# cmower/optas

Hardware: AMD Instinct MI355X
Metric: MPC solves/sec (KUKA 7-DoF, T=50) (higher is better)
Workload: dtype f64; 1 GPU; figure_eight_plan T=50 KUKA LWR end_effector_ball (BASELINE configs[1]) x 262144 perturbed instances per GPU (qc0 + U(-0.1,0.1)^7, seed=qc), solved to reduced-gradient tol 1e-08, max_iter 300; batch_per_gpu=262144, global_batch=262144, T=50, parallelism=dp1 (instances sharded, one RCCL broadcast of constants), rccl_world=1, hessian=hybrid, streams_per_gpu=2

## Files before the change

include/optas_hip.h:

```cpp
#ifndef OPTAS_HIP_H
#define OPTAS_HIP_H

#include <stddef.h>

#ifdef __cplusplus
extern "C" {
#endif

#define OH_ABI_VERSION 8

#define OH_MAX_CHAIN 16
#define OH_MAX_T 256

enum {
  OH_OK = 0,
  OH_ERR_INVALID = 1,
  OH_ERR_HIP = 2,
  OH_ERR_STATE = 3
};

enum {
  OH_STATUS_CONVERGED = 0,
  OH_STATUS_MAX_ITER = 1,
  OH_STATUS_NUMERICAL = 2,
// ... 164 lines not shown
typedef struct oh_handle oh_handle;

int oh_create(const oh_problem_desc* desc, oh_handle** out);

int oh_create_pointmass(const oh_pointmass_desc* desc, oh_handle** out);

int oh_create_qp(const oh_qp_desc* desc, oh_handle** out);

int oh_qp_set_tape(oh_handle* h, const oh_tape_desc* tape);

int oh_create_tape(const oh_tape_desc* desc, oh_handle** out);

int oh_tape_probe(oh_handle* h, int B, const double* x, const double* p, int n_regs, const int* regs, double* val, const double* seeds, double* adj,
                  double* grad);

int oh_tape_phi(oh_handle* h, int B, const double* x, const double* p, const double* lam, const double* mu, double rho, double* merit, double* f, double* rows,
                double* grad, double* cmax, double* meas);

int oh_tape_set_metric(oh_handle* h, const double* H0);

int oh_tape_compile(const oh_tape_desc* desc, size_t* code_bytes, char* source, size_t source_cap, size_t* source_len);

int oh_create_torque(const oh_torque_desc* desc, oh_handle** out);

int oh_create_ik(const oh_ik_desc* desc, oh_handle** out);

int oh_set_constants(oh_handle* h, const oh_chain* chain);
int oh_set_constants_device(oh_handle* h, const void* d_chain, size_t nbytes);

#define OH_COMM_ID_BYTES 128
int oh_comm_unique_id(char* id );
int oh_comm_init(int rank, int world, const char* id );
int oh_comm_broadcast_constants(oh_handle* h, int root);
int oh_comm_barrier(void);
int oh_comm_allreduce_max(double* value);
int oh_comm_allreduce_sum(double* value);
int oh_comm_allgather(const void* d_send, void* d_recv, size_t bytes);
int oh_comm_destroy(void);
int oh_comm_info(int* rank, int* world);
int oh_get_constants(oh_handle* h, oh_chain* out);

int oh_set_guards(oh_handle* h, const oh_guards* guards);

int oh_solve(oh_handle* h, int B, const double* x0, const double* p, double* x, double* f, double* kkt,
             int* iters, int* status);

int oh_get_flag(oh_handle* h, const char* name, int* value);

int oh_set_option(oh_handle* h, const char* name, double value);
int oh_get_option(oh_handle* h, const char* name, double* value);

int oh_max_batch(oh_handle* h, int* out);

int oh_solve_device(oh_handle* h, int B, const void* d_x0, const void* d_p, void* d_x, void* d_f, void* d_kkt,
                    void* d_iters, void* d_status);

int oh_pm_rollout(oh_handle* h, int B, int n_ticks, int advance, double ramp, const double* state0, const double* obs_table, double* states,
                  double* f, int* iters, int* status);

int oh_tq_rollout(oh_handle* h, int B, int n_ticks, int advance, double mu_warm, const double* state0, const double* goal_table, double* states,
                  double* tau0, double* f, int* iters, int* status);

int oh_get_multipliers(oh_handle* h, int B, double* lam_h);

int oh_fk_jac(oh_handle* h, int N, const double* q, double* pose, double* J);
int oh_fk_jac_device(oh_handle* h, int N, const void* d_q, void* d_pose, void* d_J);

int oh_set_dynamics(oh_handle* h, const oh_dynamics* dyn);
int oh_rnea(oh_handle* h, int N, const double* q, const double* qd, const double* qdd, double* tau);
int oh_rnea_device(oh_handle* h, int N, const void* d_q, const void* d_qd, const void* d_qdd, void* d_tau);
int oh_rnea_jac(oh_handle* h, int N, const double* q, const double* qd, const double* qdd, double* J);
int oh_rnea_hess(oh_handle* h, int N, const double* q, const double* qd, const double* qdd, const double* c, double* H);

int oh_fk_jac_soa_device(oh_handle* h, int N, const void* d_q, void* d_pose, void* d_J);

typedef struct oh_link_out {
  double *pos, *rot, *quat, *rpy, *axis, *Jg, *Ja;
} oh_link_out;
int oh_set_link_frames(oh_handle* h, const oh_chain* link, const oh_chain* base);
int oh_link_kin(oh_handle* h, int N, const double* q, const double* axis3, const oh_link_out* out);
int oh_link_kin_device(oh_handle* h, int N, const void* d_q, const double* axis3, const oh_link_out* d_out_soa);

int oh_set_profiling(oh_handle* h, int enable);
int oh_get_timing(oh_handle* h, double* out11);

enum { OH_SPECIALIZE_NEVER = 0, OH_SPECIALIZE_ALWAYS = 1, OH_SPECIALIZE_AUTO = 2 };
int oh_specialize(oh_handle* h);
int oh_specialize_compile(const oh_chain* chain, double* info2);
int oh_specialize_info(oh_handle* h, double* info4);
int oh_kernel_info_handle(oh_handle* h, const char* kernel, int* out5);

int oh_device_count(int* n);
int oh_set_device(int index);
int oh_device_malloc(void** ptr, size_t nbytes);
int oh_device_free(void* ptr);
int oh_memcpy_h2d(void* dst, const void* src, size_t nbytes);
int oh_memcpy_d2h(void* dst, const void* src, size_t nbytes);
int oh_device_synchronize(void);
int oh_event_timer_start(oh_handle* h);
int oh_event_timer_stop(oh_handle* h, double* ms);

int oh_kernel_info(const char* kernel, int* out5);

const char* oh_last_error(void);
const char* oh_version(void);
int oh_abi_version(void);
void oh_destroy(oh_handle* h);

#ifdef __cplusplus
}
#endif
#endif
```

optas_amd/backend.py:

```python
from __future__ import annotations

import ctypes as C
import os
from dataclasses import dataclass
from typing import Optional

import numpy as np

from . import _lib


@dataclass
class BatchResult:
    x: np.ndarray
    f: np.ndarray
    kkt: np.ndarray
    iters: np.ndarray
    status: np.ndarray


class _OptionsMixin:

    def set_option(self, name: str, value: float):
        _lib.set_option(self._h, name, value)
        return self

    def set_options(self, options=None, **kw):
        for k, v in {**(options or {}), **kw}.items():
            self.set_option(k, v)
        return self

    def get_option(self, name: str) -> float:
        return _lib.get_option(self._h, name)


class _SolveMixin(_OptionsMixin):

    def solve(self, x0: np.ndarray, p: np.ndarray) -> "BatchResult":
        lib = _lib.load()
        x0 = _lib.as_f64(x0)
        p = _lib.as_f64(p)
        if x0.ndim == 1:
            x0 = x0.reshape(1, -1)
        if p.ndim == 1:
            p = p.reshape(1, -1)
        B = x0.shape[0]
        assert x0.shape == (B, self.nx), f"x0 must be (B, {self.nx})"
        assert p.shape == (B, self.np_), f"p must be (B, {self.np_})"
        chunk = getattr(self, "max_batch", None)
        if chunk and B > chunk:
            parts = [self.solve(x0[i : i + chunk], p[i : i + chunk]) for i in range(0, B, chunk)]
            return BatchResult(*(np.concatenate([getattr(r, k) for r in parts]) for k in ("x", "f", "kkt", "iters", "status")))
        x = np.empty((B, self.nx))
        f = np.empty(B)
        kkt = np.empty((B, 3))
        iters = np.empty(B, dtype=np.int32)
        status = np.empty(B, dtype=np.int32)
        _lib.check(
            lib.oh_solve(self._h, B, _lib._ptr(x0), _lib._ptr(p), _lib._ptr(x), _lib._ptr(f), _lib._ptr(kkt), _lib._ptr(iters), _lib._ptr(status)),
            "oh_solve",
        )
        return BatchResult(x, f, kkt, iters, status)

    def solve_device(self, B: int, d_x0, d_p, d_x, d_f, d_kkt, d_iters, d_status) -> None:
        g = lambda b: None if b is None else b.ptr
        _lib.check(
            _lib.load().oh_solve_device(self._h, int(B), g(d_x0), g(d_p), g(d_x), g(d_f), g(d_kkt), g(d_iters), g(d_status)),
            "oh_solve_device",
        )

    def solve_ms(self) -> float:
        out = (C.c_double * 11)()
        _lib.check(_lib.load().oh_get_timing(self._h, out), "oh_get_timing")
        return out[4]

    def set_profiling(self, on: bool) -> None:
        _lib.check(_lib.load().oh_set_profiling(self._h, 1 if on else 0), "oh_set_profiling")

    def close(self) -> None:
        if getattr(self, "_h", None):
            _lib.load().oh_destroy(self._h)
            self._h = None

    def __del__(self):
        try:
            self.close()
        except Exception:
            pass


class PointMassBackend(_SolveMixin):

    def __init__(self, T=20, dt=0.05, w_acc=0.0025 / 20, ylim=1.5, vlim=1.0, safe=0.3, max_iter=100, tol=1e-8, track_final_only=False, w_vel=0.0,
                 fix_final_velocity=False):
        lib = _lib.load()
        self.T = int(T)
        self.nx, self.np_ = 4 * self.T, 4 + 4 * self.T
        desc = _lib.oh_pointmass_desc(T=self.T, dt=float(dt), w_acc=float(w_acc), ylim=float(ylim), vlim=float(vlim), safe=float(safe),
                                      max_iter=int(max_iter), tol=float(tol), track_final_only=1 if track_final_only else 0, w_vel=float(w_vel),
                                      fix_final_velocity=1 if fix_final_velocity else 0)
        self._h = C.c_void_p()
        _lib.check(lib.oh_create_pointmass(C.byref(desc), C.byref(self._h)), "oh_create_pointmass")

    def rollout(self, state0: np.ndarray, obs_table: np.ndarray, n_ticks: int, advance: int = 2, ramp: float = 0.032):
        state0 = _lib.as_f64(state0).reshape(-1, 4)
        B = state0.shape[0]
        need = n_ticks * advance + self.T
        obs_table = _lib.as_f64(obs_table).reshape(-1, 2)
        assert obs_table.shape[0] >= need, f"obs_table needs {need} rows"
        obs_table = np.ascontiguousarray(obs_table[:need])
        states = np.empty((n_ticks + 1, B, 4))
        f = np.empty((n_ticks, B))
        iters = np.empty((n_ticks, B), dtype=np.int32)
        status = np.empty((n_ticks, B), dtype=np.int32)
        _lib.check(
            _lib.load().oh_pm_rollout(self._h, B, int(n_ticks), int(advance), float(ramp), _lib._ptr(state0), _lib._ptr(obs_table), _lib._ptr(states),
                                      _lib._ptr(f), _lib._ptr(iters), _lib._ptr(status)),
            "oh_pm_rollout",
        )
        return states, f, iters, status


class TapeBackend(_SolveMixin):

    def __init__(self, tape, max_iter=2000, tol=1e-6, tol_feas=1e-9, rho0=10.0, jit=True, wave=True, options=None, keep_regs=None, metric=False):
        self.nx, self.np_ = int(tape.nx), max(1, int(tape.np_))
        self.kept_regs = None if keep_regs is None else np.asarray(keep_regs, dtype=np.int32)
        self._np_real = int(tape.np_)
        self._h = None
        self._h0 = None
        if isinstance(metric, np.ndarray):
            self._h0 = np.ascontiguousarray(metric, dtype=np.float64).reshape(self.nx, self.nx)
        elif metric and int(tape.nx) > 48 and int((options or {}).get("tape_lbfgs", -1)) != 0:
            from .tape import quadratic_cost_metric

            self._h0 = quadratic_cost_metric(tape)
        want_wave = bool(wave) and int(tape.nx) > 48 and float((options or {}).get("tape_wave", 1)) != 0.0
        if want_wave:
            from .tape import Tape, rebalance_sums

            if keep_regs is None:
                bal, kept = rebalance_sums(tape), None
            else:
                nk = len(self.kept_regs)
                tmp = rebalance_sums(Tape(tape.op, tape.a, tape.b, tape.c, tape.out_cost, np.concatenate([tape.out_rows, self.kept_regs]).astype(np.int32),
                                          tape.n_ineq, tape.n_eq + nk, tape.nx, tape.np_))
                bal = Tape(tmp.op, tmp.a, tmp.b, tmp.c, tmp.out_cost, tmp.out_rows[: len(tmp.out_rows) - nk].copy(), tape.n_ineq, tape.n_eq, tape.nx, tape.np_)
                kept = np.asarray(tmp.out_rows[len(tmp.out_rows) - nk :], dtype=np.int32)
            self._create(bal, max_iter, tol, tol_feas, rho0, jit, options)
            if self.flag("tape_wave") == 0:
                self.close()
                want_wave = False
            elif kept is not None:
                self.kept_regs = kept
        if not want_wave:
# ... 216 lines not shown
                               np.asarray(M, dtype=np.float64).reshape(-1), np.asarray(c, dtype=np.float64).reshape(-1),
                               np.asarray(A, dtype=np.float64).reshape(-1), np.asarray(b, dtype=np.float64).reshape(-1)])

    def multipliers(self, B: int):
        out = np.empty((B, self.m + self.me))
        if self.m + self.me:
            _lib.check(_lib.load().oh_get_multipliers(self._h, int(B), _lib._ptr(out)), "oh_get_multipliers")
        return out[:, : self.m], out[:, self.m :]


class IKBackend(_SolveMixin):

    def __init__(self, chain: _lib.oh_chain, lo, up, w_nominal=1.0, max_iter=200, tol=1e-6, tol_feas=1e-9, rho0=0.0):
        lib = _lib.load()
        self.ndof = int(chain.ndof)
        self.nx, self.np_ = self.ndof, self.ndof + 3
        desc = _lib.oh_ik_desc(ndof=self.ndof, w_nominal=float(w_nominal), max_iter=int(max_iter), tol=float(tol), tol_feas=float(tol_feas),
                               rho0=float(rho0))
        lo, up = np.asarray(lo, dtype=np.float64).reshape(-1), np.asarray(up, dtype=np.float64).reshape(-1)
        assert lo.shape == (self.ndof,) and up.shape == (self.ndof,)
        for i in range(self.ndof):
            desc.q_lo[i], desc.q_up[i] = lo[i], up[i]
        self._h = C.c_void_p()
        _lib.check(lib.oh_create_ik(C.byref(desc), C.byref(self._h)), "oh_create_ik")
        _lib.check(lib.oh_set_constants(self._h, C.byref(chain)), "oh_set_constants")
        self.chain = chain

    def multipliers(self, B: int):
        out = np.empty((B, 3 + 2 * self.ndof))
        _lib.check(_lib.load().oh_get_multipliers(self._h, int(B), _lib._ptr(out)), "oh_get_multipliers")
        return out[:, :3], out[:, 3 : 3 + self.ndof], out[:, 3 + self.ndof :]


def tape_default_max_iter(nx: int) -> int:
    return 2000 if nx <= 48 else 500000


class TorqueBackend(_SolveMixin):

    def __init__(self, chain: _lib.oh_chain, dynamics: _lib.oh_dynamics, T=30, dt=0.1, w_path=1000.0, w_vel=0.1, w_tau=1e-4, tau_lo=None, tau_up=None,
                 max_iter=300, tol=1e-6, tol_compl=1e-8, mu_barrier0=0.0, mu0=0.0, dq_lo=None, dq_up=None):
        lib = _lib.load()
        self.ndof, self.T = int(chain.ndof), int(T)
        self.nx, self.np_ = 4 * self.ndof * self.T, 2 * self.ndof + 3 * self.T
        self.vel = dq_lo is not None
        desc = _lib.oh_torque_desc(T=self.T, ndof=self.ndof, dt=float(dt), w_path=float(w_path), w_vel=float(w_vel), w_tau=float(w_tau),
                                   max_iter=int(max_iter), tol=float(tol), tol_compl=float(tol_compl), mu_barrier0=float(mu_barrier0), mu0=float(mu0),
                                   vel_limits=1 if self.vel else 0)
        lo = np.broadcast_to(np.asarray(-1e9 if tau_lo is None else tau_lo, dtype=np.float64), (self.ndof,))
        up = np.broadcast_to(np.asarray(1e9 if tau_up is None else tau_up, dtype=np.float64), (self.ndof,))
        for i in range(self.ndof):
            desc.tau_lo[i], desc.tau_up[i] = lo[i], up[i]
        if self.vel:
            vlo = np.broadcast_to(np.asarray(dq_lo, dtype=np.float64), (self.ndof,))
            vup = np.broadcast_to(np.asarray(dq_up, dtype=np.float64), (self.ndof,))
            for i in range(self.ndof):
                desc.dq_lo[i], desc.dq_up[i] = vlo[i], vup[i]
        self._h = C.c_void_p()
        _lib.check(lib.oh_create_torque(C.byref(desc), C.byref(self._h)), "oh_create_torque")
        _lib.check(lib.oh_set_constants(self._h, C.byref(chain)), "oh_set_constants")
        _lib.check(lib.oh_set_dynamics(self._h, C.byref(dynamics)), "oh_set_dynamics")
        self.chain, self.dynamics = chain, dynamics

    def multipliers(self, B: int):
        out = np.empty((B, self.T, (4 if self.vel else 2) * self.ndof))
        _lib.check(_lib.load().oh_get_multipliers(self._h, int(B), _lib._ptr(out)), "oh_get_multipliers")
        return out

    def rollout(self, state0, goal_table, n_ticks: int, advance: int = 1, mu_warm: float = 1e-6):
        state0 = _lib.as_f64(state0).reshape(-1, 2 * self.ndof)
        B = state0.shape[0]
        goal_table = _lib.as_f64(goal_table)
        assert goal_table.shape == (B, n_ticks * advance + self.T, 3), goal_table.shape
        states = np.empty((n_ticks + 1, B, 2 * self.ndof))
        tau0 = np.empty((n_ticks, B, self.ndof))
        f = np.empty((n_ticks, B))
        iters = np.empty((n_ticks, B), dtype=np.int32)
        status = np.empty((n_ticks, B), dtype=np.int32)
        _lib.check(_lib.load().oh_tq_rollout(self._h, B, int(n_ticks), int(advance), float(mu_warm), _lib._ptr(state0), _lib._ptr(goal_table), _lib._ptr(states),
                                             _lib._ptr(tau0), _lib._ptr(f), _lib._ptr(iters), _lib._ptr(status)), "oh_tq_rollout")
        return states, tau0, f, iters, status

    def timing(self) -> dict:
        out = (C.c_double * 11)()
        _lib.check(_lib.load().oh_get_timing(self._h, out), "oh_get_timing")
        return {"solve_ms": out[4], "iterations_launched": int(out[5]), "work_instances": out[6], "eval_ms": out[0], "step_ms": out[2]}


class FigureEightBackend(_OptionsMixin):

    def __init__(
        self,
        chain: _lib.oh_chain,
        T: int,
        dt: float,
        local_path: np.ndarray,
        w_path: float = 1000.0,
        w_vel: float = 0.01,
        max_iter: int = 200,
        tol: float = 1e-6,
        tol_feas: float = 1e-9,
        hessian: int = _lib.OH_HESSIAN_HYBRID,
        mu0: float = 0.0,
        lock_orientation: bool = True,
        fix_dq0: bool = True,
        path_in_frame: bool = True,
        guards: "Optional[_lib.oh_guards]" = None,
        ndof: Optional[int] = None,
    ):
        lib = _lib.load()
        if chain is None:
            assert ndof is not None, "a handle without constants needs ndof"
            chain_arg, chain = None, _lib.oh_chain(ndof=int(ndof))
        else:
            chain_arg = chain
        self.T, self.ndof = int(T), int(chain.ndof)
        self.nx = self.ndof * self.T + self.ndof * (self.T - 1)
        self.np_ = self.ndof + (1 + self.T if chain.has_lead else 0)
        lp = _lib.as_f64(local_path, (self.T, 3))
        self._lp = lp
        desc = _lib.oh_problem_desc(
            kind=_lib.OH_PROBLEM_FIGURE_EIGHT,
            T=self.T,
            ndof=self.ndof,
            dt=float(dt),
            w_path=float(w_path),
            w_vel=float(w_vel),
            local_path=lp.ctypes.data_as(C.POINTER(C.c_double)),
            lock_orientation=1 if lock_orientation else 0,
            fix_dq0=1 if fix_dq0 else 0,
            path_in_frame=1 if path_in_frame else 0,
            max_iter=int(max_iter),
            tol=float(tol),
            tol_feas=float(tol_feas),
            hessian=int(hessian),
            mu0=float(mu0),
        )
        self._h = C.c_void_p()
        _lib.check(lib.oh_create(C.byref(desc), C.byref(self._h)), "oh_create")
        mb = C.c_int(0)
        _lib.check(lib.oh_max_batch(self._h, C.byref(mb)), "oh_max_batch")
        self.max_batch = (mb.value // 65536) * 65536 if mb.value >= 65536 else (mb.value or None)
        if chain_arg is not None:
            _lib.check(lib.oh_set_constants(self._h, C.byref(chain)), "oh_set_constants")
        self.chain = chain_arg
        self.guards = guards
        self.n_rows = 0
        if guards is not None:
            _lib.check(lib.oh_set_guards(self._h, C.byref(guards)), "oh_set_guards")
            self.np_ = self.ndof + guards.n_links + 4 * guards.n_obstacles
            self.n_rows = (2 * self.ndof if guards.limits else 0) + guards.n_links * guards.n_obstacles + (2 * self.ndof if guards.vel_limits else 0)

    @property
    def handle(self) -> C.c_void_p:
        return self._h

    def set_constants_device(self, dptr: int, nbytes: int) -> None:
        _lib.check(_lib.load().oh_set_constants_device(self._h, C.c_void_p(dptr), nbytes), "oh_set_constants_device")

    def constants(self) -> _lib.oh_chain:
        out = _lib.oh_chain()
        _lib.check(_lib.load().oh_get_constants(self._h, C.byref(out)), "oh_get_constants")
        return out

    def solve(self, x0: np.ndarray, p: np.ndarray) -> BatchResult:
        lib = _lib.load()
        x0 = _lib.as_f64(x0)
        p = _lib.as_f64(p)
        if x0.ndim == 1:
            x0 = x0.reshape(1, -1)
        if p.ndim == 1:
            p = p.reshape(1, -1)
        B = x0.shape[0]
        assert x0.shape == (B, self.nx), f"x0 must be (B, {self.nx})"
        assert p.shape == (B, self.np_), f"p must be (B, {self.np_})"
        chunk = getattr(self, "max_batch", None)
        if chunk and B > chunk:
            parts, lams, tms = [], [], []
            for i in range(0, B, chunk):
                parts.append(self.solve(x0[i : i + chunk], p[i : i + chunk]))
                lams.append(self.multipliers(len(parts[-1].f)))
                tms.append(self.timing())
            self._chunked = {"B": B, "lam": np.concatenate(lams), "timing": {k: type(tms[0][k])(sum(t[k] for t in tms)) for k in tms[0]}}
            return BatchResult(*(np.concatenate([getattr(r, k) for r in parts]) for k in ("x", "f", "kkt", "iters", "status")))
        self._chunked = None
        x = np.empty((B, self.nx))
        f = np.empty(B)
        kkt = np.empty((B, 3))
        iters = np.empty(B, dtype=np.int32)
        status = np.empty(B, dtype=np.int32)
        _lib.check(
            lib.oh_solve(self._h, B, _lib._ptr(x0), _lib._ptr(p), _lib._ptr(x), _lib._ptr(f), _lib._ptr(kkt), _lib._ptr(iters), _lib._ptr(status)),
            "oh_solve",
        )
        return BatchResult(x, f, kkt, iters, status)

    def solve_device(self, B: int, d_x0, d_p, d_x, d_f, d_kkt, d_iters, d_status) -> None:
        g = lambda b: None if b is None else b.ptr
        self._chunked = None
        _lib.check(
            _lib.load().oh_solve_device(self._h, int(B), g(d_x0), g(d_p), g(d_x), g(d_f), g(d_kkt), g(d_iters), g(d_status)),
            "oh_solve_device",
        )

    def multipliers(self, B: int) -> np.ndarray:
        ch = getattr(self, "_chunked", None)
        if ch is not None:
            if int(B) != ch["B"]:
                raise ValueError(f"multipliers({B}) after a chunked solve of {ch['B']} instances")
            return ch["lam"]
        lam = np.empty((B, self.T, self.n_rows)) if self.guards is not None else np.empty((B, 4 * self.T))
        _lib.check(_lib.load().oh_get_multipliers(self._h, int(B), _lib._ptr(lam)), "oh_get_multipliers")
        return lam

    def specialize(self) -> dict:
        _lib.check(_lib.load().oh_specialize(self._h), "oh_specialize")
        return self.specialize_info()

    def specialize_info(self) -> dict:
        info = (C.c_double * 4)()
        _lib.check(_lib.load().oh_specialize_info(self._h, info), "oh_specialize_info")
        return {"loaded": bool(info[0]), "fk_jac_loaded": bool(info[1]), "seconds": info[2], "from_disk_cache": bool(info[3])}

    def kernel_info(self, name: str) -> dict:
        out = (C.c_int * 5)()
        _lib.check(_lib.load().oh_kernel_info_handle(self._h, name.encode(), out), "oh_kernel_info_handle")
        v, sc, lds, blk, nb = list(out)
        return {"registers_per_lane": v, "scratch_bytes_per_lane": sc, "lds_bytes_per_block": lds, "block": blk, "blocks_per_cu": nb, "waves_per_simd": nb * blk / 64.0 / 4.0}

    def set_profiling(self, on: bool) -> None:
        _lib.check(_lib.load().oh_set_profiling(self._h, 1 if on else 0), "oh_set_profiling")

    def flag(self, name: str) -> int:
        v = C.c_int(0)
        _lib.check(_lib.load().oh_get_flag(self._h, name.encode(), C.byref(v)), "oh_get_flag")
        return v.value

    def timing(self) -> dict:
        ch = getattr(self, "_chunked", None)
        if ch is not None:
            return dict(ch["timing"])
        out = (C.c_double * 11)()
        _lib.check(_lib.load().oh_get_timing(self._h, out), "oh_get_timing")
        return {
            "eval_ms": out[0],
            "eval_launches": int(out[1]),
            "step_ms": out[2],
            "step_launches": int(out[3]),
            "solve_ms": out[4],
            "iterations_launched": int(out[5]),
            "instance_launches": int(out[6]),
            "compactions": int(out[7]),
            "couple_ms": out[8],
            "rejected_steps": int(out[9]),
            "tail_iterations": int(out[10]),
        }

    def fk_jac_soa_device(self, n: int, d_q, d_pose, d_J) -> None:
        g = lambda b: None if b is None else b.ptr
        _lib.check(_lib.load().oh_fk_jac_soa_device(self._h, int(n), g(d_q), g(d_pose), g(d_J)), "oh_fk_jac_soa_device")

    def fk_jac_device(self, n: int, d_q, d_pose, d_J) -> None:
        g = lambda b: None if b is None else b.ptr
        _lib.check(_lib.load().oh_fk_jac_device(self._h, int(n), g(d_q), g(d_pose), g(d_J)), "oh_fk_jac_device")

    def event_timer_start(self) -> None:
        _lib.check(_lib.load().oh_event_timer_start(self._h), "oh_event_timer_start")

    def event_timer_stop(self) -> float:
        ms = C.c_double(0.0)
        _lib.check(_lib.load().oh_event_timer_stop(self._h, C.byref(ms)), "oh_event_timer_stop")
        return ms.value

    def close(self) -> None:
        if self._h:
            _lib.load().oh_destroy(self._h)
            self._h = None

    def __del__(self):
        try:
            self.close()
        except Exception:
            pass


def _offsets(container) -> dict:
    if hasattr(container, "offsets"):
        return container.offsets()
    out, o = {}, 0
    for k, v in container.items():
        out[k] = o
        o += int(v.shape[0]) * int(v.shape[1])
    return out


class MultiArmBackend:

    def __init__(self, spec, opt, max_iter=200, tol=1e-6, hessian=_lib.OH_HESSIAN_GAUSS_NEWTON):
        self.spec, self.opt = spec, opt
        self.nx, self.np_ = opt.nx, opt.np
        self.xoff, self.poff = _offsets(opt.decision_variables), _offsets(opt.parameters)
        self.arms = []
        for a in spec.arms:
            guards = None
            if a.guards is not None:
                gs = a.guards
                guards = _lib.oh_guards()
                guards.limits = 1 if gs.lo is not None else 0
                if gs.lo is not None:
                    for j in range(a.robot.ndof):
                        guards.q_lo[j], guards.q_up[j] = float(gs.lo[j]), float(gs.up[j])
                if gs.vlo is not None:
                    guards.vel_limits = 1
                    for j in range(a.robot.ndof):
                        guards.dq_lo[j], guards.dq_up[j] = float(gs.vlo[j]), float(gs.vup[j])
                guards.n_links, guards.n_obstacles = len(gs.links), len(gs.obstacles)
                for l, (k, off) in enumerate(a.robot.link_attachments(a.link, gs.links)):
                    if k < 0:
                        raise NotImplementedError(f"sphere link '{gs.links[l]}' does not move with any joint of the chain to '{a.link}'")
                    guards.link_joint[l] = k
                    for i in range(3):
                        guards.link_offset[l][i] = float(off[i])
            be = FigureEightBackend(
                a.robot.kinematic_chain(a.link), spec.T, spec.dt, a.offsets, w_path=a.w_path, w_vel=a.w_vel, max_iter=max_iter, tol=tol,
                hessian=hessian, lock_orientation=False, fix_dq0=False, path_in_frame=False, guards=guards,
            )
            self.arms.append((a, be))

    def solve(self, x0: np.ndarray, p: np.ndarray) -> BatchResult:
        x0 = _lib.as_f64(x0).reshape(-1, self.nx)
        p = _lib.as_f64(p).reshape(-1, self.np_)
        B = x0.shape[0]
        x = np.empty((B, self.nx))
        f = np.zeros(B)
        kkt = np.zeros((B, 3))
        iters = np.zeros(B, dtype=np.int32)
        status = np.zeros(B, dtype=np.int32)
        for a, be in self.arms:
# ... 30 lines not shown
```

optas_amd/csrc/oh_api.hip:

```cpp
#include <algorithm>
#include <chrono>
#include <cmath>
#include <cstdlib>
#include <cstring>
#include <string>
#include <thread>
#include <utility>
#include <vector>

#include "oh_handle.h"

static thread_local std::string g_err;

int fail(int code, const std::string& msg) {
  g_err = msg;
  return code;
}

extern "C" int oh_specialize(oh_handle* h);
static bool spec_applies(const oh_handle* h);
static bool spec_tail_vel_applies(const oh_handle* h);
extern "C" const char* oh_last_error(void) { return g_err.c_str(); }
extern "C" const char* oh_version(void) { return "optas_hip 0.2 (gfx950)"; }
extern "C" int oh_abi_version(void) { return OH_ABI_VERSION; }

struct FieldOpt {
  const char* name;
  int Sched::*i;
  double Sched::*d = nullptr;
  bool flag = false;
  double get(const Sched& s) const { return d ? s.*d : s.*i; }
  void set(Sched& s, const double v) const { if (d) s.*d = v; else s.*i = flag ? v != 0.0 : (int)v; }
};
static const FieldOpt FIELD_OPTS[] = {
    {"tail_threshold", &Sched::tail_threshold}, {"free_pcr_max", &Sched::free_pcr_max}, {"compaction", &Sched::compaction, nullptr, true},
    {"compact_frac", nullptr, &Sched::compact_frac}, {"compact_sort", &Sched::compact_sort}, {"compact_carry", &Sched::compact_carry},
    {"compact_fused", &Sched::compact_fused, nullptr, true},
    {"tail_vel", &Sched::tail_vel}, {"lg_split", &Sched::lg_split}, {"tail_vel_threshold", &Sched::tail_vel_threshold},
    {"fuse_couple", &Sched::fuse_couple, nullptr, true}, {"sparse_check_below", &Sched::sparse_check_below}, {"specialize", &Sched::specialize},
    {"tq_check", &Sched::tq_check},
};
static const FieldOpt* field_opt(const std::string& name) {
  for (const FieldOpt& f : FIELD_OPTS)
    if (name == f.name) return &f;
  return nullptr;
}
static int set_option_impl(oh_handle* h, const std::string& name, double v) {
  Sched& sc = h->sch;
  if (name == "compact_frac") sc.compact_frac = sc.compact_frac_restart = v;
  else if (name == "specialize") sc.specialize = v == 0.0 ? OH_SPECIALIZE_NEVER : (v == 1.0 ? OH_SPECIALIZE_ALWAYS : OH_SPECIALIZE_AUTO);
  else if (name == "tq_check") sc.tq_check = v >= 1.0 ? (int)v : 1;
  else if (name == "batch_invariant") {
    const bool was = batch_invariant(h) != 0.0;
    h->opt[name] = v;
    if (v != 0.0 && !was) {
      sc.inv_saved = {sc.compaction ? 1.0 : 0.0, (double)sc.tail_threshold, (double)sc.tail_vel, h->opt.count("free_persist") ? h->opt["free_persist"] : -2.0};
      sc.compaction = false; sc.tail_threshold = 0; sc.tail_vel = 0; h->opt["free_persist"] = 0;
    } else if (v == 0.0 && was) {
      sc.compaction = sc.inv_saved[0] != 0.0; sc.tail_threshold = (int)sc.inv_saved[1]; sc.tail_vel = (int)sc.inv_saved[2];
      if (sc.inv_saved[3] == -2.0) h->opt.erase("free_persist"); else h->opt["free_persist"] = sc.inv_saved[3];
    }
  } else if (const FieldOpt* f = field_opt(name)) f->set(sc, v);
  else {
    bool known = false;
    for (const OptDoc& d : OPT_TABLE) known = known || name == d.name;
    if (!known) return fail(OH_ERR_INVALID, "oh_set_option: unknown option '" + name + "'");
    h->opt[name] = v;
    if (h->desc.kind == OH_PROBLEM_TAPE && !h->tape.h_op.empty() && name.rfind("tape_", 0) == 0 && name != "tape_lds_max") return tape_configure(h);
  }
  return OH_OK;
}
extern "C" int oh_set_option(oh_handle* h, const char* name, double value) {
  if (!h || !name) return fail(OH_ERR_INVALID, "oh_set_option: null argument");
  return set_option_impl(h, name, value);
}
extern "C" int oh_get_option(oh_handle* h, const char* name, double* value) {
  if (!h || !name || !value) return fail(OH_ERR_INVALID, "oh_get_option: null argument");
  const std::string n(name);
  if (n == "batch_invariant") *value = batch_invariant(h);
  else if (const FieldOpt* f = field_opt(n)) *value = f->get(h->sch);
  else {
    for (const OptDoc& d : OPT_TABLE)
      if (n == d.name) { *value = opt_value(h, d); return OH_OK; }
    return fail(OH_ERR_INVALID, "oh_get_option: unknown option '" + n + "'");
  }
  return OH_OK;
}
static int apply_debug_options(oh_handle* h) {
  const char* e = getenv("OH_DEBUG_OPTIONS");
  if (!e || !*e) return OH_OK;
  std::string str(e);
  size_t pos = 0;
  while (pos < str.size()) {
    size_t end = str.find_first_of(",;", pos);
    if (end == std::string::npos) end = str.size();
    const std::string item = str.substr(pos, end - pos);
    pos = end + 1;
    if (item.empty()) continue;
    const size_t eq = item.find('=');
    if (eq == std::string::npos) return fail(OH_ERR_INVALID, "OH_DEBUG_OPTIONS: expected name=value, got '" + item + "'");
    char* endp = nullptr;
    const std::string val = item.substr(eq + 1);
    const double v = strtod(val.c_str(), &endp);
    if (endp == val.c_str()) return fail(OH_ERR_INVALID, "OH_DEBUG_OPTIONS: '" + item + "' has no numeric value");
    if (const int rc = set_option_impl(h, item.substr(0, eq), v)) return rc;
  }
  return OH_OK;
}
static oh_handle* new_handle() {
  oh_handle* h = new oh_handle();
  if (apply_debug_options(h) != OH_OK) {
    delete h;
    return nullptr;
  }
  return h;
}

oh_handle* open_handle(const std::string& who, const int kind, const int T, const int ndof, const int want, int* rc) {
  int nd = 0;
  if (hipGetDeviceCount(&nd) != hipSuccess || nd < 1) {
    *rc = fail(OH_ERR_HIP, who + ": no HIP device available (this library has no CPU path)");
    return nullptr;
  }
  oh_handle* h = new_handle();
  if (!h) {
    *rc = OH_ERR_INVALID;
    return nullptr;
  }
  h->desc = oh_problem_desc{};
  h->desc.kind = kind;
  h->desc.T = T;
  h->desc.ndof = ndof;
  hipGetDevice(&h->device);
  bool ok = hipStreamCreate(&h->stream) == hipSuccess;
  for (hipEvent_t* e : {&h->ev0, &h->ev1, &h->evt0, &h->evt1}) ok = ok && hipEventCreate(e) == hipSuccess;
  if ((want & OPEN_CHAIN) && ok) ok = h->d_chain.reserve(1) == hipSuccess;
  if ((want & OPEN_FLAG) && ok) ok = h->h_flag.reserve(1) == hipSuccess;
  if (!ok) {
    delete h;
    *rc = fail(OH_ERR_HIP, who + (want ? ": stream/event/allocation failed" : ": stream/event creation failed"));
    return nullptr;
  }
  return h;
}

void reset_counters(oh_handle* h) {
  for (double& t : h->timing) t = 0.0;
  h->timing_couple = h->rejects = h->tail_iters = 0.0;
}
int finish_solve(oh_handle* h, const double launched) {
  HIPCHK(hipEventRecord(h->ev1, h->stream));
  HIPCHK(hipStreamSynchronize(h->stream));
  HIPCHK(hipGetLastError());
  float ms = 0.f;
  HIPCHK(hipEventElapsedTime(&ms, h->ev0, h->ev1));
  reset_counters(h);
  h->timing[4] = ms;
  h->timing[5] = launched;
  return OH_OK;
}

extern "C" int oh_device_count(int* n) {
  if (!n) return fail(OH_ERR_INVALID, "oh_device_count: null");
  int c = 0;
  hipError_t e = hipGetDeviceCount(&c);
  if (e != hipSuccess) {
    *n = 0;
    return fail(OH_ERR_HIP, std::string("hipGetDeviceCount: ") + hipGetErrorString(e));
  }
  *n = c;
  return OH_OK;
}
extern "C" int oh_set_device(int index) {
  HIPCHK(hipSetDevice(index));
  return OH_OK;
}
extern "C" int oh_device_malloc(void** ptr, size_t nbytes) {
  if (!ptr) return fail(OH_ERR_INVALID, "oh_device_malloc: null");
  HIPCHK(hipMalloc(ptr, nbytes ? nbytes : 8));
  return OH_OK;
}
extern "C" int oh_device_free(void* ptr) {
  HIPCHK(hipFree(ptr));
  return OH_OK;
}
extern "C" int oh_memcpy_h2d(void* dst, const void* src, size_t nbytes) {
  HIPCHK(hipMemcpy(dst, src, nbytes, hipMemcpyHostToDevice));
  return OH_OK;
}
extern "C" int oh_memcpy_d2h(void* dst, const void* src, size_t nbytes) {
  HIPCHK(hipMemcpy(dst, src, nbytes, hipMemcpyDeviceToHost));
  return OH_OK;
}
extern "C" int oh_device_synchronize(void) {
  HIPCHK(hipDeviceSynchronize());
  return OH_OK;
}

extern "C" int oh_create(const oh_problem_desc* desc, oh_handle** out) {
  if (!desc || !out) return fail(OH_ERR_INVALID, "oh_create: null argument");
  *out = nullptr;
  if (desc->kind != OH_PROBLEM_FIGURE_EIGHT && desc->kind != OH_PROBLEM_KINEMATICS)
    return fail(OH_ERR_INVALID, "oh_create: unknown problem kind");
  if (desc->kind == OH_PROBLEM_KINEMATICS) {
    if (desc->ndof < 1 || desc->ndof > OH_MAX_CHAIN) return fail(OH_ERR_INVALID, "oh_create: ndof must be in [1, OH_MAX_CHAIN]");
    int rc = OH_OK;
    oh_handle* hk = open_handle("oh_create", desc->kind, desc->T, desc->ndof, OPEN_CHAIN, &rc);
    if (!hk) return rc;
    hk->desc = *desc;
    hk->desc.local_path = nullptr;
    *out = hk;
    return OH_OK;
  }
  if (desc->T < 3 || desc->T > OH_MAX_T) return fail(OH_ERR_INVALID, "oh_create: T must be in [3, OH_MAX_T]");
  if (desc->ndof < (desc->lock_orientation ? 4 : 2) || desc->ndof > 8)
    return fail(OH_ERR_INVALID, "oh_create: the trajectory kernels are instantiated for 2 ... 8 actuated joints, the orientation-locked ones (three rows per "
                                "knot, null space of ndof - 3 dimensions) for 4 ... 8");
  if (!(desc->dt > 0.0)) return fail(OH_ERR_INVALID, "oh_create: dt must be positive");
  if (!desc->local_path) return fail(OH_ERR_INVALID, "oh_create: local_path is null");
  if (desc->hessian != OH_HESSIAN_GAUSS_NEWTON && desc->hessian != OH_HESSIAN_EXACT && desc->hessian != OH_HESSIAN_HYBRID)
    return fail(OH_ERR_INVALID, "oh_create: bad hessian mode");
  int rc = OH_OK;
  oh_handle* h = open_handle("oh_create", desc->kind, desc->T, desc->ndof, OPEN_CHAIN | OPEN_FLAG, &rc);
  if (!h) return rc;
  h->desc = *desc;
  h->local_path.assign(desc->local_path, desc->local_path + 3 * (size_t)desc->T);
  h->desc.local_path = nullptr;
  if (h->desc.max_iter <= 0) h->desc.max_iter = 200;
  if (!(h->desc.tol > 0.0)) h->desc.tol = 1e-6;
  if (!(h->desc.tol_feas > 0.0)) h->desc.tol_feas = 1e-9;
  if (h->desc.mu0 < 0.0) h->desc.mu0 = 0.0;
// ... 236 lines not shown
  P.al_fuse = (int)optv(h, "al_fuse");
  P.local_path = h->d_local_path;
  P.np = (int)shape_of(h).npar;
  P.zc = (h->sch.fuse_couple && d.lock_orientation && !h->have_guards && !h->chain_host.has_lead) ? 1 : 0;
  P.zc_free = (h->sch.fuse_couple && !d.lock_orientation && !(h->have_guards && h->guards.vel_limits)) ? 1 : 0;
}

__global__ __launch_bounds__(256) static void k_gather_int(const int* __restrict__ src, int* __restrict__ dst, const int B, const int* __restrict__ newidx) {
  const int b = blockIdx.x * blockDim.x + threadIdx.x;
  if (b < B && newidx[b] >= 0) dst[newidx[b]] = src[b];
}
static int move_everything(oh_handle* h, hipStream_t s, int Bnew) {
  const int N = h->desc.ndof, NZ = N - 3, T = h->desc.T, Bp = h->D.Bp, B = h->D.B;
  FigBuffers& D = h->D;
  GuardBuffers& GB = h->GB;
  const GuardParams& GP = h->GP;
  struct Item { void* p; int rows; bool is_int; };
  std::vector<Item> items;
  auto dbl = [&](double* p, int rows) { if (p) items.push_back({p, rows, false}); };
  auto itg = [&](int* p) { if (p) items.push_back({p, 1, true}); };
  const bool zc = h->P.zc != 0, slim = optv(h, "invariant_move_slim") != 0.0;
  struct Pair { double* a0; double* a1; int rows; };
  std::vector<Pair> live;
  const bool live_only = zc && !h->have_guards && optv(h, "invariant_move_live") != 0.0;
  if (live_only) {
    live.push_back({D.Z[0], D.Z[1], T * (3 * N - 3)}); live.push_back({D.Dr[0], D.Dr[1], T * (NZ * (NZ + 1) / 2)}); live.push_back({D.g[0], D.g[1], T * N});
    live.push_back({D.cv[0], D.cv[1], T}); live.push_back({D.Gfull[0], D.Gfull[1], T * N}); live.push_back({D.mdl[0], D.mdl[1], T * (3 + 3 * NZ)});
    live.push_back({D.merit[0], D.merit[1], T});
  }
  for (int sl = 0; sl < 2; ++sl) {
    dbl(D.q[sl], T * N);
    if (!live_only) {
      dbl(D.Z[sl], T * (3 * N - 3)); dbl(D.Dr[sl], T * (NZ * (NZ + 1) / 2)); dbl(D.g[sl], T * N); dbl(D.cv[sl], T);
      dbl(D.Gfull[sl], T * N); dbl(D.mdl[sl], T * (3 + 3 * NZ)); dbl(D.merit[sl], T);
    }
    if (!(zc && slim)) { dbl(D.phi[sl], T); dbl(D.E[sl], T * NZ * NZ); dbl(D.gt[sl], T * NZ); }
    dbl(GB.psi[sl], T); dbl(GB.mcv[sl], T);
  }
  dbl(D.zstep, T * NZ); dbl(D.ref, 12);
  if (!(zc && slim)) { dbl(D.Kmat, T * NZ * NZ); dbl(D.kvec, T * NZ); }
  if (h->chain_host.has_lead || !slim) dbl(D.lead, T);
  for (double* p : {D.fconst, D.f_cur, D.pred, D.mu, D.nun, D.stat, D.feas, D.fpsi, GB.rho, GB.rho_next, GB.omega, GB.meas_prev, GB.meas, GB.ls_gd, GB.ls_q}) dbl(p, 1);
  dbl(GB.lam, T * GP.NC); dbl(GB.lamv, GP.vel ? T * 2 * N : 0); dbl(GB.par, GP.n_links + 4 * GP.n_obs);
  for (int* p : {D.cur, D.first, D.skip, D.polish, D.stale, D.status, D.iters, D.orig, GB.outer, GB.n_outer, GB.ls_count}) itg(p);
  int max_rows = 1;
  for (const Item& it : items) max_rows = it.rows > max_rows ? it.rows : max_rows;
  for (const Pair& pr : live) max_rows = pr.rows > max_rows ? pr.rows : max_rows;
  const size_t need = sizeof(double) * ((size_t)max_rows + 1) * Bp;
  HIPCHK(h->move_scr.reserve(need));
  if (!live.empty()) {
    int* curn = (int*)((double*)h->move_scr.p + (size_t)max_rows * Bp);
    hipLaunchKernelGGL(k_gather_int, dim3((B + 255) / 256), dim3(256), 0, s, (const int*)D.cur, curn, B, (const int*)D.newidx);
    for (const Pair& pr : live) oh_launch_move_rows_live(s, pr.a0, pr.a1, (double*)h->move_scr.p, pr.rows, Bp, B, Bnew, D.newidx, D.cur, curn);
  }
  for (const Item& it : items) oh_launch_move_rows(s, it.p, h->move_scr.p, it.rows, Bp, B, Bnew, D.newidx, it.is_int);
  return OH_OK;
}

static int ensure_peers(oh_handle* h, const int n) {
  const bool tqk = h->desc.kind == OH_PROBLEM_TORQUE_MPC;
  HIPCHK(hipSetDevice(h->device));
  while ((int)h->peers.size() < n) {
    oh_handle* p = nullptr;
    int rc;
    if (tqk) rc = oh_create_torque(&h->tq.desc, &p);
    else {
      oh_problem_desc d = h->desc;
      d.local_path = h->local_path.data();
      rc = oh_create(&d, &p);
    }
    if (rc) return rc;
    p->is_peer = true;
    p->device = h->device;
    rc = oh_set_constants(p, &h->chain_host);
    if (!rc && tqk) rc = oh_set_dynamics(p, &h->dyn_host);
    if (!rc && !tqk && h->have_guards) rc = oh_set_guards(p, &h->guards);
    if (rc) { delete p; return rc; }
    h->peers.push_back(p);
  }
  return OH_OK;
}
static int solve_device(oh_handle* h, const Solve& a, bool may_fan_out, LastSolve* rec);
struct Tally {
  double launched = 0, work = 0, compactions = 0, rejects = 0, tails = 0;
};
static int lane_solve(oh_handle* q, Tally& t, const Solve& a) {
  if (const int rc = solve_device(q, a, false, nullptr)) return rc;
  t.launched = std::max(t.launched, q->timing[5]);
  t.work += q->timing[6];
  t.compactions += q->timing[7];
  t.rejects += q->rejects;
  t.tails += q->tail_iters;
  return OH_OK;
}
template <class Work>
static int fan_out(oh_handle* h, const int n, Work&& work) {
  if (const int rc = ensure_peers(h, n - 1)) return rc;
  for (int i = 0; i + 1 < n; ++i) {
    oh_handle* p = h->peers[i];
    p->sch = h->sch;
    p->opt = h->opt;
    p->spec = h->spec;
    p->spec_failed = h->spec_failed;
    p->spec_cache_checked = true;
  }
  std::vector<int> rcs(n, OH_OK);
  std::vector<std::string> errs(n);
  std::vector<Tally> tally(n);
  auto lane = [&](const int i) {
    oh_handle* q = i == 0 ? h : h->peers[i - 1];
    if (hipSetDevice(h->device) != hipSuccess) rcs[i] = fail(OH_ERR_HIP, "hipSetDevice failed on a lane's host thread");
    else rcs[i] = work(i, q, tally[i]);
    if (rcs[i]) errs[i] = oh_last_error();
  };
  const auto t0 = std::chrono::steady_clock::now();
  std::vector<std::thread> th;
  for (int i = 1; i < n; ++i) th.emplace_back(lane, i);
  lane(0);
  for (std::thread& t : th) t.join();
  const double ms = std::chrono::duration<double, std::milli>(std::chrono::steady_clock::now() - t0).count();
  for (int i = 0; i < n; ++i)
    if (rcs[i]) return fail(rcs[i], errs[i]);
  reset_counters(h);
  h->timing[4] = ms;
  for (const Tally& t : tally) {
    h->timing[5] = std::max(h->timing[5], t.launched);
    h->timing[6] += t.work;
    h->timing[7] += t.compactions;
    h->rejects += t.rejects;
    h->tail_iters += t.tails;
  }
  return OH_OK;
}
static int solve_split(oh_handle* h, const int S, const Solve& a, LastSolve* rec) {
  const Shape sh = shape_of(h);
  std::vector<int> lo(S + 1, 0);
  for (int i = 1; i <= S; ++i) lo[i] = (int)((long long)a.B * i / S / 64 * 64);
  lo[S] = a.B;
  std::vector<LastSolve::Part> parts(S);
  const int rc = fan_out(h, S, [&](const int i, oh_handle* q, Tally& t) {
    parts[i] = {q, lo[i + 1] - lo[i]};
    return lane_solve(q, t, a.part((size_t)lo[i], parts[i].n, sh));
  });
  if (rc) return rc;
  rec->parts = parts;
  return OH_OK;
}

struct Traj {
  int B, N, NV, check_every, hard_cap;
  bool guarded, lead, prof, invariant;
  const FigSpec* spec;
  FreeSweep sweep;
  const double* p;
  double *x, *f, *kkt;
  int *iters, *status;
  int launched, compactions;
  size_t ne;
};
static FreeSweep free_sweep(oh_handle* h, const int nb, const bool start = false) {
  const int N = h->desc.ndof, nK = h->desc.T - h->P.t0;
  FreeSweep sw = FREE_SERIAL;
  if (!h->P.lock && batch_invariant(h) == 0.0 && nb <= h->sch.free_pcr_max && nK <= 128 && (N == 6 || N == 7)) {
    if (N == 7 && (int)optv(h, "free_bb") != 0) sw = FREE_BB;
    else sw = (nb <= (int)optv(h, "free_cp_max") && nK <= 64) ? FREE_CP : FREE_PCR;
  }
  if (!start) return sw;
  h->P.inst_major = sw == FREE_BB ? 1 : 0;
  const int fp = (int)optv(h, "free_persist");
  const bool fits = (nK <= 64 && nb <= 512) || fp == 1;
  return (sw == FREE_BB && h->have_guards && !h->GP.vel && h->P.zc_free && !h->profiling && fits && fp != 0) ? FREE_PERSIST : sw;
}
static int mark(oh_handle* h, Traj& r, const int tag, const size_t room = 2) {
  if (!r.prof || r.ne + room >= h->prof_events.size()) return OH_OK;
  size_t& ne = r.ne;
  hipStream_t s = h->stream;
  HIPCHK(hipEventRecord(h->prof_events[ne++], s));
  h->prof_tags.push_back(tag);
  return OH_OK;
}
static bool check_after(const oh_handle* h, const Traj& r, const int it, const bool tail_ok) {
  return (it + 1) % ((!tail_ok && r.check_every == 1 && h->D.B <= h->sch.sparse_check_below) ? 8 : r.check_every) == 0;
}
static int look(oh_handle* h, const bool check, int* nrun) {
  *nrun = -1;
  if (!check) return OH_OK;
  hipStream_t s = h->stream;
  HIPCHK(hipMemcpyAsync(h->h_flag, h->D.n_running, sizeof(int), hipMemcpyDeviceToHost, s));
  HIPCHK(hipStreamSynchronize(s));
  *nrun = *h->h_flag;
  return OH_OK;
}
static void finalize(oh_handle* h, const Traj& r, const int only_done) {
  hipStream_t s = h->stream;
  if (r.spec && r.spec->finalize) {
    oh_launch_finalize(s, r.N, h->P, h->D, only_done, r.x, r.f, r.kkt, r.iters, r.status, 1);
    if (oh_spec_launch_finalize(*r.spec, s, h->P, h->D, only_done, r.f, r.kkt, r.iters, r.status) == hipSuccess) return;
    (void)hipGetLastError();
    oh_launch_finalize(s, r.N, h->P, h->D, only_done, r.x, r.f, r.kkt, r.iters, r.status, 2);
    return;
  }
  oh_launch_finalize(s, r.N, h->P, h->D, only_done, r.x, r.f, r.kkt, r.iters, r.status);
}
static int compact_batch(oh_handle* h, Traj& r, const int nrun, const int slot, const bool move) {
  hipStream_t s = h->stream;
  finalize(h, r, 1);
  if (r.guarded) oh_launch_guard_emit(s, h->P, h->D, h->GP, h->GB, r.NV, 1);
  oh_launch_scan_running(s, h->D, h->sch.compact_sort);
  if (move) {
    if (const int rc = move_everything(h, s, nrun)) return rc;
  } else {
    oh_launch_compact(s, r.N, h->P, h->D, 0, 0, 0);
    if (r.guarded) oh_launch_guard_compact(s, h->P, h->D, h->GP, h->GB, r.NV, 0, 0);
    oh_launch_compact(s, r.N, h->P, h->D, 1, nrun, slot);
    if (r.guarded) oh_launch_guard_compact(s, h->P, h->D, h->GP, h->GB, r.NV, 1, nrun);
  }
  h->D.B = nrun;
  ++r.compactions;
  return OH_OK;
}
static int traj_prologue(oh_handle* h, Traj& r, const double* x0) {
  if (const int rc = ensure_capacity(h, r.B)) return rc;
  fill_params(h);
  if ((spec_applies(h) || spec_tail_vel_applies(h)) && !h->spec && !h->spec_failed) {
    bool want = h->sch.specialize == OH_SPECIALIZE_ALWAYS || (h->sch.specialize == OH_SPECIALIZE_AUTO && r.B >= h->specialize_min_B);
    if (!want && h->sch.specialize == OH_SPECIALIZE_AUTO && !h->spec_cache_checked) {
      h->spec_cache_checked = true;
      want = oh_jit_figure8_cached(h->chain_host, h->desc.ndof);
    }
    if (want && oh_specialize(h) != OH_OK) h->spec_failed = true;
  }
  if (r.lead && (r.guarded || !h->desc.lock_orientation || h->desc.ndof != 6))
    return fail(OH_ERR_INVALID, "oh_solve_device: a parameterised lead joint is lowered for the orientation-locked family with 6 optimised joints, "
                                "without inequality rows");
  if (!r.guarded) h->D.fpsi = nullptr;
  else if (const int rc = ensure_guards(h)) return rc;
  r.sweep = free_sweep(h, r.B, true);
  r.NV = (r.guarded && h->GP.vel) ? 2 * r.N : 0;
  r.spec = spec_applies(h) ? h->spec : nullptr;
  r.check_every = optv(h, "check_every") >= 1.0 ? (int)optv(h, "check_every") : 1;
  r.hard_cap = 2 * h->desc.max_iter + 2 + 40 + 64;
  hipStream_t s = h->stream;
  if (r.prof) {
    const size_t need = 4 * (size_t)(2 * h->desc.max_iter + 44) + 64;
    while (h->prof_events.size() < need) {
      hipEvent_t e;
      HIPCHK(hipEventCreate(&e));
      h->prof_events.push_back(e);
    }
  }
  HIPCHK(hipEventRecord(h->ev0, s));
  HIPCHK(hipMemsetAsync(h->D.work, 0, 4 * sizeof(unsigned long long), s));
  if (!oh_launch_setup(s, r.N, h->P, h->D, x0, r.p)) return fail(OH_ERR_INVALID, "oh_solve_device: unsupported ndof");
  if (r.guarded) oh_launch_setup_guards(s, r.N, h->P, h->D, h->GP, h->GB, r.p);
  h->prof_tags.clear();
  return mark(h, r, 0);
}
static bool launch_tail(oh_handle* h, const Traj& r, const bool tail_vel, const int slot) {
  hipStream_t s = h->stream;
  if (tail_vel && h->spec && spec_tail_vel_applies(h)) return oh_spec_launch_tail_vel(*h->spec, s, h->P, h->D, h->GP, h->GB, slot) == hipSuccess;
  if (tail_vel) return oh_launch_tail_vel(s, r.N, h->P, h->D, h->GP, h->GB, slot);
  if (r.spec) return oh_spec_launch_tail(*r.spec, s, h->P, h->D, slot) == hipSuccess;
  return oh_launch_tail(s, r.N, h->P, h->D, slot);
}
static void launch_eval(oh_handle* h, const Traj& r, const int slot, const int part) {
  if (!r.spec) oh_launch_eval(h->stream, r.N, h->P, h->D, slot, part);
  else oh_spec_launch_eval(*r.spec, h->stream, h->P, h->D, slot, part);
}

static int locked_loop(oh_handle* h, Traj& r) {
  FigParams& P = h->P; FigBuffers& D = h->D; const GuardParams& GP = h->GP; const GuardBuffers& GB = h->GB;
  const hipStream_t s = h->stream;
  const int N = r.N;
  const bool tail_vel = r.guarded && (GP.vel || GP.limits) && GP.n_links == 0 && h->sch.tail_vel;
  const bool tail_ok = (h->desc.T - P.t0 <= 64) && h->sch.tail_threshold > 0 && (!r.guarded || tail_vel) && !r.lead;
  const int tail_threshold = tail_vel ? h->sch.tail_vel_threshold : h->sch.tail_threshold;
  if (tail_ok && r.B <= tail_threshold) {
    if (!launch_tail(h, r, tail_vel, 0)) return fail(OH_ERR_INVALID, "oh_solve_device: no persistent kernel for this handle (ndof / rows)");
    return OH_OK;
  }
  const bool lg_split = r.guarded && h->sch.lg_split && GP.n_links == 0, lg_spec = lg_split && h->spec && spec_tail_vel_applies(h);
  const bool couple_vel = !P.zc && r.guarded && GP.vel, couple = !P.zc && !couple_vel;
  const bool carry = h->sch.compaction && h->sch.compact_carry && (size_t)h->desc.T * ((N - 3) * (N - 2) / 2) >= 22 && !r.guarded && !r.lead;
  const double inv_frac = optv(h, "invariant_compact_frac");
  const bool inv_move = r.invariant && !r.lead && inv_frac > 0.0, restart = h->sch.compaction && !r.lead, restart_moves = r.guarded && optv(h, "compact_move_all") != 0.0;
  int nrun = -1, carry_pending = 0;
  for (int it = 0; it < r.hard_cap; ++it) {
    if (nrun >= 0)
      if (const int rc = mark(h, r, 0, 3)) return rc;
    const int slot = it & 1;
    if (lg_split) {
      if (!(lg_spec && oh_spec_launch_eval(*h->spec, s, P, D, slot, 1) == hipSuccess)) oh_launch_eval_locked_guarded(s, N, P, D, GP, GB, slot, 1);
      oh_launch_eval_locked_guarded(s, N, P, D, GP, GB, slot, 2);
    } else if (r.guarded) oh_launch_eval_locked_guarded(s, N, P, D, GP, GB, slot, 0);
    else if (r.lead) oh_launch_eval_lead(s, N, P, D, slot);
    else if (carry_pending > 0) {
      bool moved = false, scanned = false;
      if (r.spec && r.spec->retract_move && h->sch.compact_fused && !h->spec_move_failed) {
        finalize(h, r, 1);
        oh_launch_scan_running(s, D, h->sch.compact_sort);
        scanned = true;
        if (const int rc = mark(h, r, 0)) return rc;
        moved = oh_spec_launch_eval(*r.spec, s, P, D, slot, 3) == hipSuccess;
        if (moved) {
          if (const int rc = mark(h, r, 4)) return rc;
          oh_launch_carry(s, N, P, D, 2, 0, slot);
        } else {
          (void)hipGetLastError();
          h->spec_move_failed = true;
        }
      }
      if (!moved) {
        launch_eval(h, r, slot, 1);
        if (const int rc = mark(h, r, 4)) return rc;
        if (!scanned) {
          finalize(h, r, 1);
          oh_launch_scan_running(s, D, h->sch.compact_sort);
        }
        oh_launch_carry(s, N, P, D, 0, 0, slot);
      }
      oh_launch_carry(s, N, P, D, 1, carry_pending, slot);
      std::swap(D.q[slot], D.q_spare[0]);
      std::swap(D.q[1 - slot], D.q_spare[1]);
      if (P.hessian != OH_HESSIAN_GAUSS_NEWTON || P.zc) std::swap(D.Gfull[1 - slot], D.G_spare);
      D.B = carry_pending;
      carry_pending = 0;
      ++r.compactions;
      if (const int rc = mark(h, r, 0)) return rc;
      launch_eval(h, r, slot, 2);
    } else launch_eval(h, r, slot, 0);
    if (const int rc = mark(h, r, 1)) return rc;
    if (couple_vel) oh_launch_couple_vel(s, N, P, D, GP, GB, slot);
    else if (couple) oh_launch_couple(s, N, P, D, slot);
    const bool check = check_after(h, r, it, tail_ok);
    if (const int rc = mark(h, r, 3)) return rc;
    if (r.guarded) oh_launch_step_locked_guarded(s, N, P, D, GP, GB, slot);
    else oh_launch_step(s, N, P, D, slot);
    if (const int rc = mark(h, r, 2)) return rc;
    ++r.launched;
    if (const int rc = look(h, check, &nrun)) return rc;
    if (nrun == 0) break;
    if (tail_ok && nrun > 0 && nrun <= tail_threshold) {
      if (const int rc = compact_batch(h, r, nrun, (it + 1) & 1, false)) return rc;
      if (!launch_tail(h, r, tail_vel, (it + 1) & 1)) return fail(OH_ERR_INVALID, "oh_solve_device: no persistent kernel for this handle (ndof / rows)");
      break;
    }
    if (nrun < 0 || D.B < 512) continue;
    if (carry && (double)nrun <= h->sch.compact_frac * (double)D.B) {
      carry_pending = nrun;
    } else if (inv_move && (double)nrun <= inv_frac * (double)D.B) {
      if (const int rc = compact_batch(h, r, nrun, 0, true)) return rc;
      if (const int rc = mark(h, r, 0)) return rc;
    } else if (restart && (double)nrun <= h->sch.compact_frac_restart * (double)D.B) {
      if (const int rc = compact_batch(h, r, nrun, (it + 1) & 1, restart_moves)) return rc;
      if (const int rc = mark(h, r, 0)) return rc;
    }
  }
  return OH_OK;
}
static int free_loop(oh_handle* h, Traj& r) {
  FigParams& P = h->P; FigBuffers& D = h->D; const GuardParams& GP = h->GP; const GuardBuffers& GB = h->GB;
  const hipStream_t s = h->stream;
  const int N = r.N;
  FreeSweep sweep = r.sweep;
  h->free_sweep_last = (int)sweep;
  h->free_sweeps_used = 1 << (int)sweep;
  if (sweep == FREE_PERSIST) {
    if (!oh_launch_free_persist(s, N, P, D, GP, GB)) return fail(OH_ERR_INVALID, "oh_solve_device: no persistent kernel for this handle (ndof / rows)");
    r.launched = 1;
    return OH_OK;
  }
  const bool couple_vel = !P.zc_free && r.guarded && GP.vel, couple = !P.zc_free && !couple_vel;
  int nrun = -1;
  for (int it = 0; it < r.hard_cap; ++it) {
    if (nrun >= 0)
      if (const int rc = mark(h, r, 0, 3)) return rc;
    const int slot = it & 1;
    if (r.guarded) oh_launch_eval_guarded(s, N, P, D, GP, GB, slot);
    else oh_launch_eval_free(s, N, P, D, slot);
    if (const int rc = mark(h, r, 1)) return rc;
    if (couple_vel) oh_launch_couple_free_vel(s, N, P, D, GP, GB, slot);
    else if (couple) oh_launch_couple_free(s, N, P, D, slot);
    const bool check = check_after(h, r, it, false);
    if (check) HIPCHK(hipMemsetAsync(h->D.n_running, 0, sizeof(int), s));
    if (const int rc = mark(h, r, 3)) return rc;
    if (r.guarded) oh_launch_step_guarded(s, N, P, D, GP, GB, slot, sweep);
    else oh_launch_step_free(s, N, P, D, slot, sweep);
    if (const int rc = mark(h, r, 2)) return rc;
    ++r.launched;
    if (const int rc = look(h, check, &nrun)) return rc;
    if (nrun == 0) break;
    if (nrun > 0 && h->sch.compaction && D.B >= 512 && (double)nrun <= h->sch.compact_frac_restart * (double)D.B) {
      if (const int rc = compact_batch(h, r, nrun, (it + 1) & 1, false)) return rc;
      sweep = free_sweep(h, D.B);
      h->free_sweeps_used |= 1 << (int)sweep;
      if (const int rc = mark(h, r, 0)) return rc;
    }
  }
  return OH_OK;
}
static int traj_epilogue(oh_handle* h, Traj& r) {
  hipStream_t s = h->stream;
  finalize(h, r, 0);
  if (r.guarded) oh_launch_guard_emit(s, h->P, h->D, h->GP, h->GB, r.NV, 0);
  h->D.B = r.B;
  if (r.guarded) oh_launch_guard_infeasible(s, r.N, h->P, h->D, h->GP, r.p, r.B, r.kkt, r.status);
  if (const int frc = finish_solve(h, r.launched)) return frc;
  unsigned long long work[3] = {0, 0, 0};
  HIPCHK(hipMemcpyAsync(work, h->D.work, sizeof(work), hipMemcpyDeviceToHost, s));
  HIPCHK(hipStreamSynchronize(s));
  h->timing[6] = (double)work[0];
  h->rejects = (double)work[1];
  h->tail_iters = (double)work[2];
  if (r.prof) {
    double ms[4] = {0, 0, 0, 0};
    int n[5] = {0, 0, 0, 0, 0};
    for (size_t i = 1; i < r.ne; ++i) {
      const int tag = h->prof_tags[i];
      float m = 0.f;
      if (tag) hipEventElapsedTime(&m, h->prof_events[i - 1], h->prof_events[i]);
      ms[tag == 4 ? 1 : tag] += m;
      ++n[tag];
    }
    h->timing[0] = ms[1]; h->timing[1] = n[1]; h->timing[2] = ms[2]; h->timing[3] = n[2]; h->timing_couple = ms[3];
  }
  h->timing[7] = r.compactions;
  return OH_OK;
}
static int traj_solve_device(oh_handle* h, const Solve& a) {
  Traj r{};
  r.B = a.B; r.N = h->desc.ndof;
  r.guarded = h->have_guards; r.lead = h->chain_host.has_lead != 0; r.prof = h->profiling; r.invariant = batch_invariant(h) != 0.0;
  r.p = a.p; r.x = a.x; r.f = a.f; r.kkt = a.kkt; r.iters = a.iters; r.status = a.status;
  if (const int rc = traj_prologue(h, r, a.x0)) return rc;
  if (const int rc = h->P.lock ? locked_loop(h, r) : free_loop(h, r)) return rc;
  return traj_epilogue(h, r);
}

static int split_parts(const oh_handle* h, const int B, const bool may_fan_out) {
  const int S = std::min(8, (int)optv(h, "streams"));
  if (!may_fan_out || h->profiling || S < 2) return 1;
  if (h->desc.kind == OH_PROBLEM_TORQUE_MPC) return (B >= (int)optv(h, "tq_split_min") && B / S >= 64 && h->have_chain && h->have_dyn) ? S : 1;
  if (spec_applies(h) && (batch_invariant(h) == 0.0 || optv(h, "invariant_split") != 0.0) && B >= (int)optv(h, "split_min") && B / S >= 4096 && stage_fits(h, B))
    return S;
  return (!h->desc.lock_orientation && !h->chain_host.has_lead && batch_invariant(h) == 0.0 && B >= (int)optv(h, "free_split_min") && B / S >= 64) ? S : 1;
}

static int solve_device(oh_handle* h, const Solve& a, const bool may_fan_out, LastSolve* rec) {
  const int B = a.B;
  if (B < 1) return fail(OH_ERR_INVALID, "oh_solve_device: B must be >= 1");
  if (!a.x0 || !a.p) return fail(OH_ERR_INVALID, "oh_solve_device: x0 and p are required");
  if (rec) *rec = LastSolve{B, {{h, B}}, false};
  switch (h->desc.kind) {
    case OH_PROBLEM_POINT_MASS_MPC: return pm_solve_device(h, a);
    case OH_PROBLEM_IK: return ik_solve_device(h, a);
    case OH_PROBLEM_QP: return qp_solve_device(h, a);
    case OH_PROBLEM_TAPE: return tape_solve_device(h, a);
    case OH_PROBLEM_TORQUE_MPC: break;
    case OH_PROBLEM_FIGURE_EIGHT:
      if (!h->have_chain) return fail(OH_ERR_STATE, "oh_solve_device: call oh_set_constants first");
      if (!solver_chain_ok(h->chain_host)) return fail(OH_ERR_INVALID, "oh_solve_device: the solver needs a chain that covers every model joint in order");
      HIPCHK(hipSetDevice(h->device));
      break;
    default: return fail(OH_ERR_STATE, "oh_solve_device: handle was created without a problem (OH_PROBLEM_KINEMATICS)");
  }
  if (const int S = split_parts(h, B, may_fan_out); S > 1) {
    if (spec_applies(h) && !h->spec && !h->spec_failed && h->sch.specialize != OH_SPECIALIZE_NEVER && oh_specialize(h) != OH_OK) h->spec_failed = true;
    return solve_split(h, S, a, rec);
  }
  return h->desc.kind == OH_PROBLEM_TORQUE_MPC ? tq_solve_device(h, a) : traj_solve_device(h, a);
}

extern "C" int oh_solve_device(oh_handle* h, int B, const void* d_x0, const void* d_p, void* d_x, void* d_f, void* d_kkt,
                               void* d_iters, void* d_status) {
  if (!h) return fail(OH_ERR_INVALID, "oh_solve_device: null handle");
  h->last = LastSolve{};
  LastSolve rec;
  const Solve a{B, (const double*)d_x0, (const double*)d_p, (double*)d_x, (double*)d_f, (double*)d_kkt, (int*)d_iters, (int*)d_status};
  const int rc = solve_device(h, a, !h->is_peer, &rec);
  if (rc == OH_OK) h->last = rec;
  return rc;
}

int ensure_stage(oh_handle* h, size_t bytes) {
  const hipError_t e = h->stage.reserve(bytes);
  if (e != hipSuccess) return fail(OH_ERR_HIP, std::string("staging allocation failed: ") + hipGetErrorString(e));
  return OH_OK;
}
static int stage_solve(oh_handle* q, const Shape& sh, const size_t n, StageLayout& L) {
  return stage_carve(q, [&](Carver c) {
    layout_stage(c, L, sh, n);
    return c.bytes();
  });
}

static const double* mult_ptr(const oh_handle* q) {
// ... 64 lines not shown
extern "C" int oh_solve(oh_handle* h, int B, const double* x0, const double* p, double* x, double* f, double* kkt, int* iters,
                        int* status) {
  if (!h) return fail(OH_ERR_INVALID, "oh_solve: null handle");
  if (B < 1) return fail(OH_ERR_INVALID, "oh_solve: B must be >= 1");
  if (!x0 || !p) return fail(OH_ERR_INVALID, "oh_solve: x0 and p are required");
  if (!shape_of(h).nx) return fail(OH_ERR_STATE, "oh_solve: handle was created without a problem (OH_PROBLEM_KINEMATICS)");
  HIPCHK(hipSetDevice(h->device));
  h->last = LastSolve{};
  const bool tqk = h->desc.kind == OH_PROBLEM_TORQUE_MPC;
  const int chunk = std::max(1024, (int)optv(h, "pipe_chunk"));
  if ((h->desc.kind == OH_PROBLEM_FIGURE_EIGHT || tqk) && !h->is_peer && !h->profiling && optv(h, "pipe") != 0.0 && h->have_chain && !h->have_guards &&
      !h->chain_host.has_lead && B >= 2 * chunk && (!tqk || h->have_dyn)) {
    const int rc = solve_pipelined(h, B, chunk, x0, p, x, f, kkt, iters, status);
    if (rc == OH_OK) h->last = LastSolve{B, {}, true};
    return rc;
  }
  const Shape sh = shape_of(h);
  StageLayout L{};
  int rc = stage_solve(h, sh, (size_t)B, L);
  if (rc) return rc;
  LastSolve rec;
  const bool small = L.total <= OH_PINNED_STAGE_BYTES && (h->h_stage || h->h_stage.reserve(OH_PINNED_STAGE_BYTES) == hipSuccess);
  StageLayout M = L;
  if (small) {
    Carver mirror(h->h_stage.p, Carver::Slots);
    layout_stage(mirror, M, sh, (size_t)B);
    memcpy(M.x0, x0, L.b_x);
    memcpy(M.p, p, L.b_p);
    HIPCHK(hipMemcpy(L.x0, M.x0, L.in_bytes(), hipMemcpyHostToDevice));
  } else {
    HIPCHK(hipMemcpy(L.x0, x0, L.b_x, hipMemcpyHostToDevice));
    HIPCHK(hipMemcpy(L.p, p, L.b_p, hipMemcpyHostToDevice));
  }
  rc = solve_device(h, Solve{B, L.x0, L.p, L.x, L.f, L.kkt, L.iters, L.status}, !h->is_peer, &rec);
  if (rc) return rc;
  if (small) {
    HIPCHK(hipMemcpy(M.x, L.x, L.out_bytes(), hipMemcpyDeviceToHost));
    if (x) memcpy(x, M.x, L.b_x);
    if (f) memcpy(f, M.f, L.b_f);
    if (kkt) memcpy(kkt, M.kkt, L.b_k);
    if (iters) memcpy(iters, M.iters, L.b_i);
    if (status) memcpy(status, M.status, L.b_i);
  } else {
    if (x) HIPCHK(hipMemcpy(x, L.x, L.b_x, hipMemcpyDeviceToHost));
    if (f) HIPCHK(hipMemcpy(f, L.f, L.b_f, hipMemcpyDeviceToHost));
    if (kkt) HIPCHK(hipMemcpy(kkt, L.kkt, L.b_k, hipMemcpyDeviceToHost));
    if (iters) HIPCHK(hipMemcpy(iters, L.iters, L.b_i, hipMemcpyDeviceToHost));
    if (status) HIPCHK(hipMemcpy(status, L.status, L.b_i, hipMemcpyDeviceToHost));
  }
  h->last = rec;
  return OH_OK;
}

extern "C" int oh_get_multipliers(oh_handle* h, int B, double* lam_h) {
  if (!h || !lam_h) return fail(OH_ERR_INVALID, "oh_get_multipliers: null argument");
  const LastSolve& r = h->last;
  if (h->desc.kind == OH_PROBLEM_POINT_MASS_MPC || B != r.B || B < 1) return fail(OH_ERR_STATE, "oh_get_multipliers: B does not match the last solve");
  HIPCHK(hipSetDevice(h->device));
  const size_t per = shape_of(h).mult;
  if (!per && h->desc.kind == OH_PROBLEM_FIGURE_EIGHT) return fail(OH_ERR_STATE, "oh_get_multipliers: this problem has no nonlinear equality rows");
  if (r.pipe_cache) {
    HIPCHK(hipMemcpy(lam_h, h->d_pipe_mult, sizeof(double) * per * B, hipMemcpyDeviceToHost));
    return OH_OK;
  }
  size_t o = 0;
  for (const LastSolve::Part& part : r.parts) {
    if (const int rc = copy_multipliers(part.q, part.n, lam_h + o * per)) return rc;
    o += (size_t)part.n;
  }
  return OH_OK;
}

extern "C" int oh_set_profiling(oh_handle* h, int enable) {
  if (!h) return fail(OH_ERR_INVALID, "oh_set_profiling: null handle");
  h->profiling = enable != 0;
  return OH_OK;
}
extern "C" int oh_get_timing(oh_handle* h, double* out8) {
  if (!h || !out8) return fail(OH_ERR_INVALID, "oh_get_timing: null argument");
  for (int i = 0; i < 8; ++i) out8[i] = h->timing[i];
  out8[8] = h->timing_couple;
  out8[9] = h->rejects;
  out8[10] = h->tail_iters;
  return OH_OK;
}
extern "C" int oh_event_timer_start(oh_handle* h) {
  if (!h) return fail(OH_ERR_INVALID, "oh_event_timer_start: null handle");
  HIPCHK(hipEventRecord(h->evt0, h->stream));
  return OH_OK;
}
extern "C" int oh_event_timer_stop(oh_handle* h, double* ms) {
  if (!h || !ms) return fail(OH_ERR_INVALID, "oh_event_timer_stop: null argument");
  HIPCHK(hipEventRecord(h->evt1, h->stream));
  HIPCHK(hipEventSynchronize(h->evt1));
  float f = 0.f;
  HIPCHK(hipEventElapsedTime(&f, h->evt0, h->evt1));
  *ms = f;
  return OH_OK;
}

extern "C" void oh_destroy(oh_handle* h) {
  if (h) delete h;
}

extern "C" int oh_get_constants(oh_handle* h, oh_chain* out) {
  if (!h || !out) return fail(OH_ERR_INVALID, "oh_get_constants: null argument");
  if (!h->have_chain) return fail(OH_ERR_STATE, "oh_get_constants: no constants set");
  *out = h->chain_host;
  return OH_OK;
}

static bool spec_applies(const oh_handle* h) {
  return h->desc.kind == OH_PROBLEM_FIGURE_EIGHT && h->have_chain && h->desc.lock_orientation && !h->have_guards && !h->chain_host.has_lead;
}
static bool spec_tail_vel_applies(const oh_handle* h) {
  return h->desc.kind == OH_PROBLEM_FIGURE_EIGHT && h->have_chain && h->desc.lock_orientation && h->have_guards && !h->chain_host.has_lead &&
         (h->guards.limits || h->guards.vel_limits) && h->guards.n_links == 0 && h->sch.tail_vel;
}
extern "C" int oh_specialize(oh_handle* h) {
  if (!h) return fail(OH_ERR_INVALID, "oh_specialize: null handle");
  if (!h->have_chain) return fail(OH_ERR_STATE, "oh_specialize: call oh_set_constants first");
  HIPCHK(hipSetDevice(h->device));
  const auto t0 = std::chrono::steady_clock::now();
  int rc = specialize_fk(h);
  if (rc == OH_OK && (spec_applies(h) || spec_tail_vel_applies(h)) && !h->spec) {
    std::string err;
    const FigSpec* sp = nullptr;
    if (oh_jit_figure8(h->chain_host, h->desc.ndof, &sp, &err)) {
      h->spec_failed = true;
      rc = fail(OH_ERR_HIP, "oh_specialize: " + err);
    } else h->spec = sp;
  }
  h->spec_seconds = std::chrono::duration<double>(std::chrono::steady_clock::now() - t0).count();
  return rc;
}
extern "C" int oh_specialize_compile(const oh_chain* chain, double* info2) {
  if (!chain) return fail(OH_ERR_INVALID, "oh_specialize_compile: null chain");
  if (chain->ndof < 4 || chain->ndof > OH_MAX_CHAIN || chain->n_chain != chain->ndof || chain->has_lead)
    return fail(OH_ERR_INVALID, "oh_specialize_compile: the chain must cover every model joint in order (4..16 joints, no lead joint)");
  const auto t0 = std::chrono::steady_clock::now();
  std::vector<char> code;
  bool from_disk = false;
  std::string err;
  bool fd2 = false;
  if (oh_jit_compile_cached(oh_jit_figure8_source(*chain, chain->ndof), &code, &from_disk, &err) || oh_jit_compile_cached(oh_jit_fkjac_source(*chain), &code, &fd2, &err))
    return fail(OH_ERR_HIP, "oh_specialize_compile: " + err);
  from_disk = from_disk && fd2;
  if (info2) {
    info2[0] = std::chrono::duration<double>(std::chrono::steady_clock::now() - t0).count();
    info2[1] = from_disk ? 1.0 : 0.0;
  }
  return OH_OK;
}
extern "C" int oh_specialize_info(oh_handle* h, double* info4) {
  if (!h || !info4) return fail(OH_ERR_INVALID, "oh_specialize_info: null argument");
  info4[0] = h->spec ? 1.0 : 0.0;
  info4[1] = h->fk_spec ? 1.0 : 0.0;
  info4[2] = h->spec_seconds;
  info4[3] = ((h->spec && h->spec->from_disk) || (!h->spec && h->fk_spec && h->fk_spec->from_disk)) ? 1.0 : 0.0;
  return OH_OK;
}
extern "C" int oh_get_flag(oh_handle* h, const char* name, int* value) {
  if (!h || !name || !value) return fail(OH_ERR_INVALID, "oh_get_flag: null argument");
  const std::string n(name);
  if (n == "fuse_couple") {
    fill_params(h);
// ... 39 lines not shown
```

optas_amd/csrc/oh_carve.h:

```cpp
#pragma once
#include <cstddef>
#include <utility>
#include <vector>

#include "oh_kernels.h"

class Carver {
 public:
  enum Mode { Packed, Slots };
  Carver(void* base, const Mode mode) : base_((char*)base), mode_(mode) {}
  template <class T>
  T* take(const size_t n) {
    off_ = up(off_, mode_ == Slots ? 256 : alignof(T));
    T* const r = base_ ? (T*)(base_ + off_) : nullptr;
    if (log) log->push_back({off_, n * sizeof(T)});
    off_ += n * sizeof(T);
    return r;
  }
  size_t bytes() const { return mode_ == Slots ? up(off_, 256) : off_; }
  std::vector<std::pair<size_t, size_t>>* log = nullptr;

 private:
  static size_t up(const size_t v, const size_t a) { return (v + a - 1) / a * a; }
  char* base_;
  Mode mode_;
  size_t off_ = 0;
};


inline void layout_fig(Carver& c, FigBuffers& D, const int N, const int lock, const int T, const int Bp) {
  const int NZ = lock ? N - 3 : N;
  const size_t per_q = (size_t)T * N * Bp;
  const size_t per_Z = (size_t)T * (3 * N - 3) * Bp;
  const size_t per_Dr = (size_t)T * (NZ * (NZ + 1) / 2) * Bp;
  const size_t per_t = (size_t)T * Bp;
  for (int s = 0; s < 2; ++s) D.q[s] = c.take<double>(per_q);
  for (int s = 0; s < 2; ++s) D.q_spare[s] = c.take<double>(per_q);
  for (int s = 0; s < 2; ++s) D.Z[s] = c.take<double>(per_Z);
  for (int s = 0; s < 2; ++s) D.Dr[s] = c.take<double>(per_Dr);
  for (int s = 0; s < 2; ++s) D.g[s] = c.take<double>(per_q);
  for (int s = 0; s < 2; ++s) D.phi[s] = c.take<double>(per_t);
  for (int s = 0; s < 2; ++s) D.cv[s] = c.take<double>(per_t);
  for (int s = 0; s < 2; ++s) D.Gfull[s] = c.take<double>(per_q);
  D.G_spare = c.take<double>(per_q);
  for (int s = 0; s < 2; ++s) D.mdl[s] = c.take<double>((size_t)T * (3 + 3 * NZ) * Bp);
  for (int s = 0; s < 2; ++s) D.E[s] = c.take<double>((size_t)T * NZ * NZ * Bp);
  for (int s = 0; s < 2; ++s) D.gt[s] = c.take<double>((size_t)T * NZ * Bp);
  for (int s = 0; s < 2; ++s) D.merit[s] = c.take<double>(per_t);
  D.zstep = c.take<double>((size_t)T * NZ * Bp);
  D.Kmat = c.take<double>((size_t)T * NZ * NZ * Bp);
  D.kvec = c.take<double>((size_t)T * NZ * Bp);
  D.ref = c.take<double>((size_t)12 * Bp);
  D.fconst = c.take<double>(Bp);
  D.f_cur = c.take<double>(Bp);
  D.pred = c.take<double>(Bp);
  D.mu = c.take<double>(Bp);
  D.nun = c.take<double>(Bp);
  D.stat = c.take<double>(Bp);
  D.feas = c.take<double>(Bp);
  D.lam_h = c.take<double>((size_t)4 * T * Bp);
  D.lead = c.take<double>(per_t);
  if (!lock) D.lam_h = nullptr;
  D.cur = c.take<int>(Bp);
  D.first = c.take<int>(Bp);
  D.skip = c.take<int>(Bp);
  D.polish = c.take<int>(Bp);
  D.stale = c.take<int>(Bp);
  D.status = c.take<int>(Bp);
  D.iters = c.take<int>(Bp);
  D.orig = c.take<int>(Bp);
  D.newidx = c.take<int>(Bp);
  D.n_running = c.take<int>(1);
  D.n_new = c.take<int>(1);
  D.work = c.take<unsigned long long>(14);
  D.n_defer = D.work ? (int*)(D.work + 3) : nullptr;
  D.scan_blk = c.take<int>(8 * 1024);
  D.defer_list = c.take<int>(2 * (size_t)Bp);
  c.take<int>(2);
}

inline void layout_guards(Carver& c, GuardBuffers& GB, double*& fpsi, const GuardParams& GP, const int N, const int T, const int Bp) {
  const size_t npar = (size_t)GP.n_links + 4 * (size_t)GP.n_obs;
  const size_t n_lam = (size_t)T * GP.NC * Bp, n_lamv = GP.vel ? (size_t)T * 2 * N * Bp : 0;
  GB.lam = c.take<double>(n_lam);
  GB.par = c.take<double>(npar * Bp);
  GB.psi[0] = c.take<double>((size_t)T * Bp);
  GB.psi[1] = c.take<double>((size_t)T * Bp);
  GB.rho = c.take<double>(Bp);
  GB.rho_next = c.take<double>(Bp);
  GB.omega = c.take<double>(Bp);
  GB.meas_prev = c.take<double>(Bp);
  fpsi = c.take<double>(Bp);
  GB.mcv[0] = c.take<double>((size_t)T * Bp);
  GB.mcv[1] = c.take<double>((size_t)T * Bp);
  GB.meas = c.take<double>(Bp);
  GB.lamv = GP.vel ? c.take<double>(n_lamv) : nullptr;
  GB.lam_out = c.take<double>(n_lam);
  GB.lamv_out = GP.vel ? c.take<double>(n_lamv) : nullptr;
  GB.scr = c.take<double>(n_lam + n_lamv + (npar + 8) * Bp);
  GB.ls_gd = c.take<double>(Bp);
  GB.ls_q = c.take<double>(Bp);
  GB.outer = c.take<int>(Bp);
  GB.n_outer = c.take<int>(Bp);
  GB.ls_count = c.take<int>(Bp);
}

inline void layout_tq(Carver& c, TqBuffers& D, const int B, const int T) {
  const size_t BT = (size_t)B * T;
  D.xs = c.take<double>(2 * BT * TQ_XS);
  D.st = c.take<double>(2 * BT * TQ_SD);
  D.lam = c.take<double>(2 * BT * TQ_LAM);
  D.gains = c.take<double>(BT * TQ_GN);
  D.goal = c.take<double>(BT * 4);
  for (double** p : {&D.f_cur, &D.f_true, &D.bsum, &D.mu, &D.nun, &D.mub, &D.stat, &D.alpha, &D.qk, &D.ndx, &D.viol}) *p = c.take<double>(B);
  for (int** p : {&D.cur, &D.first, &D.curv, &D.status, &D.iters, &D.rejected, &D.n_barrier, &D.nrel, &D.n_back, &D.stall, &D.curv_age, &D.list})
    *p = c.take<int>(B);
  D.n_running = c.take<int>(1);
  D.n_list = c.take<int>(1);
  c.take<int>(14);
}

inline void layout_pm(Carver& c, PmBuffers& D, const int T, const int Bp) {
  const size_t T1 = (size_t)(T - 1), Tn = (size_t)T;
  D.a = c.take<double>(2 * T1 * Bp);
  D.X = c.take<double>(4 * Tn * Bp);
  D.s = c.take<double>(9 * Tn * Bp);
  D.lam = c.take<double>(9 * Tn * Bp);
  D.K = c.take<double>(8 * T1 * Bp);
  D.kk = c.take<double>(2 * T1 * Bp);
  D.dX = c.take<double>(4 * Tn * Bp);
  D.da = c.take<double>(2 * T1 * Bp);
}


struct Shape { size_t nx, npar, mult; };

struct StageLayout {
  double *x0, *p, *x, *f, *kkt;
  int *iters, *status;
  size_t b_x, b_p, b_f, b_k, b_i, total;
  size_t in_bytes() const { return (size_t)((char*)p - (char*)x0) + b_p; }
  size_t out_bytes() const { return (size_t)((char*)status - (char*)x) + b_i; }
};
inline void layout_stage(Carver& c, StageLayout& L, const Shape& sh, const size_t B) {
  L.b_x = sizeof(double) * sh.nx * B; L.b_p = sizeof(double) * sh.npar * B; L.b_f = sizeof(double) * B; L.b_k = sizeof(double) * 3 * B; L.b_i = sizeof(int) * B;
  L.x0 = c.take<double>(sh.nx * B);
  L.p = c.take<double>(sh.npar * B);
  L.x = c.take<double>(sh.nx * B);
  L.f = c.take<double>(B);
  L.kkt = c.take<double>(3 * B);
  L.iters = c.take<int>(B);
  L.status = c.take<int>(B);
  L.total = c.bytes();
}
```

optas_amd/csrc/oh_figure8_units.h:

```cpp
#pragma once
#include "oh_figure8.h"

#define IDX(t, K, k) (((size_t)(t) * (K) + (k)) * Bp + b)
#define KNOT(arr, t, K) rowbuf((arr) + (size_t)(t) * (K) * (size_t)Bp)
#define RB(k) ((unsigned)(k) * rowB)
#define SPARE(k) (((size_t)t * N + (k)) * Bp + nb)



template <int N>
OH_DEV void setup_unit(const FigParams& P, const FigBuffers& D, const double* __restrict__ x0, const double* __restrict__ pin, const int b, const int tt) {
  const int Bp = D.Bp;
  if (b >= D.B) {
    if (b < Bp && tt == 0) D.status[b] = OH_STATUS_CONVERGED;
    return;
  }
  const oh_chain* ch = D.chain;
  double qc[N];
#pragma unroll
  for (int j = 0; j < N; ++j) qc[j] = pin[(size_t)b * P.np + j];
#pragma unroll
  for (int j = 0; j < N; ++j) {
    const double v = (tt < P.t0) ? qc[j] : x0[(size_t)b * P.nx + (size_t)tt * N + j];
    D.q[0][IDX(tt, N, j)] = v;
    D.q[1][IDX(tt, N, j)] = (tt < P.t0) ? qc[j] : 0.0;
  }
  if (ch->has_lead) D.lead[(size_t)tt * Bp + b] = pin[(size_t)b * P.np + N + 1 + tt];
  if (tt != 0) return;
  double R[9], p[3], z[N][3], pj[N][3];
  if (ch->has_lead) {
    double Rb[9], pb[3];
    lead_base(ch, pin[(size_t)b * P.np + N], Rb, pb);
    fk_chain<N, true>(ch, qc, R, p, z, pj, Rb, pb);
  } else {
    fk_chain<N>(ch, qc, R, p, z, pj);
  }
  double e[3], t[3], Re[9];
  mv3(R, ch->p_tool, t);
  e[0] = p[0] + t[0]; e[1] = p[1] + t[1]; e[2] = p[2] + t[2];
  mm3(R, ch->R_tool, Re);
#pragma unroll
  for (int i = 0; i < 3; ++i) D.ref[(size_t)i * Bp + b] = e[i];
#pragma unroll
  for (int i = 0; i < 9; ++i) D.ref[(size_t)(3 + i) * Bp + b] = Re[i];
  double fconst = 0.0;
  for (int tf = 0; tf < P.t0 && tf < P.T; ++tf) {
    double l[3] = {P.local_path[3 * tf], P.local_path[3 * tf + 1], P.local_path[3 * tf + 2]};
    fconst += P.w_path * dot3(l, l);
  }
  D.fconst[b] = fconst;
  D.cur[b] = 1;
  D.first[b] = 1;
  D.skip[b] = 0;
  D.polish[b] = 0;
  D.stale[b] = 0;
  D.orig[b] = b;
  D.status[b] = -1;
  D.iters[b] = 0;
  D.f_cur[b] = 0.0;
  D.pred[b] = 0.0;
  D.mu[b] = P.mu0;
  D.nun[b] = 2.0;
  D.stat[b] = 0.0;
  D.feas[b] = 0.0;
}

#ifndef OH_CHAIN
#define OH_CHAIN(D) ((D).chain)
#endif
#ifndef OH_RETRACT_PREFETCH
#define OH_RETRACT_PREFETCH 0
#endif
#ifndef OH_EVALB_PREFETCH_G
#define OH_EVALB_PREFETCH_G 1
#endif
#ifndef OH_ZC_EARLY
#define OH_ZC_EARLY 1
#endif
template <int N>
OH_DEV void load_householder(const double* __restrict__ Vs, const int Bp, const int b, const int t, double (&V)[3][N]) {
#pragma unroll
  for (int m = 0; m < 3; ++m)
#pragma unroll
    for (int k = 0; k < N; ++k) V[m][k] = (k < m) ? 0.0 : Vs[IDX(t, HV_ROWS(N), HV_OFF(N, m) + k - m)];
}

template <int N, bool GUARD = false, bool LEAD = false, int MODE = EVAL_FUSED, bool ZC = false, bool SPH = true, bool MOVE = false>
OH_DEV void eval_unit(const FigParams& P, const FigBuffers& D, const int slot, const int b, const int t, const GuardParams* GPp = nullptr,
                      const GuardBuffers* GBp = nullptr) {
  static_assert(!ZC || (MODE == EVAL_ONLY && !GUARD && !LEAD), "the folded coupling belongs to the plain batched evaluation");
  static_assert(!MOVE || (MODE == EVAL_RETRACT_ONLY && !GUARD && !LEAD), "the moving retraction belongs to the plain batched retraction");
  constexpr int NZ = N - 3;
  constexpr int NP = NZ * (NZ + 1) / 2;
  const int Bp = D.Bp;
  if (b >= D.B) return;
  const int cur = 1 - slot;
  const int status_b = D.status[b], skip_b = D.skip[b], first_b = D.first[b];
  const bool asis = (MODE == EVAL_RETRACT_ONLY && !GUARD) ? D.polish[b] == 2 : false;
  const double stat_b = D.stat[b], pred_b = D.pred[b];
  int nb = 0;
  if constexpr (MOVE) nb = D.newidx[b];
  const bool move_G = MOVE && (P.hessian != OH_HESSIAN_GAUSS_NEWTON || P.zc);
  double Gmv[N];
  constexpr bool EARLY = MODE == EVAL_ONLY || OH_RETRACT_PREFETCH;
  double Rc[9], pc[3];
  if constexpr (EARLY) {
#pragma unroll
    for (int i = 0; i < 3; ++i) pc[i] = D.ref[(size_t)i * Bp + b];
#pragma unroll
    for (int i = 0; i < 9; ++i) Rc[i] = D.ref[(size_t)(3 + i) * Bp + b];
  }
  double q[N], e_tgt[3] = {0.0, 0.0, 0.0};
  double sm_zc = 0.0;
  double zs[NZ], Vc[3][N], mdlc[3 + 3 * NZ];
  double Gpre[N];
  constexpr bool PRE_G = OH_EVALB_PREFETCH_G && MODE == EVAL_ONLY && !GUARD;
  if constexpr (MODE == EVAL_ONLY) {
#pragma unroll
    for (int j = 0; j < N; ++j) q[j] = D.q[slot][IDX(t, N, j)];
    if constexpr (PRE_G) {
      if (P.hessian != OH_HESSIAN_GAUSS_NEWTON) {
#pragma unroll
        for (int k = 0; k < N; ++k) Gpre[k] = D.Gfull[cur][IDX(t, N, k)];
      }
    }
  } else if constexpr (OH_RETRACT_PREFETCH) {
#pragma unroll
    for (int a = 0; a < NZ; ++a) zs[a] = D.zstep[IDX(t, NZ, a)];
    load_householder<N>(D.Z[cur], Bp, b, t, Vc);
#pragma unroll
    for (int j = 0; j < N; ++j) q[j] = D.q[cur][IDX(t, N, j)];
#pragma unroll
    for (int i = 0; i < 3 + 3 * NZ; ++i) mdlc[i] = D.mdl[cur][IDX(t, MDL_ROWS(N), i)];
    if constexpr (MOVE) {
      if (move_G) {
#pragma unroll
        for (int k = 0; k < N; ++k) Gmv[k] = D.Gfull[cur][IDX(t, N, k)];
      }
    }
  }
  double cpl_zc[N];
  if constexpr (ZC && OH_ZC_EARLY) {
    const double* __restrict__ qs = D.q[slot];
    const bool lastk = (t == P.T - 1);
    double qm[N], qp[N];
#pragma unroll
    for (int k = 0; k < N; ++k) {
      qm[k] = qs[IDX(t - 1, N, k)];
      qp[k] = lastk ? 0.0 : qs[IDX(t + 1, N, k)];
    }
    oh_fence(q[N - 1]);
    oh_fence(Rc[8]);
    oh_fence(qp[N - 1]);
    const double kap2 = 2.0 * P.kappa;
#pragma unroll
    for (int k = 0; k < N; ++k) {
      const double dm = q[k] - qm[k];
      sm_zc += dm * dm;
      double c = kap2 * dm;
      if (!lastk) c -= kap2 * (qp[k] - q[k]);
      cpl_zc[k] = c;
    }
  } else if constexpr (EARLY) {
    oh_fence(q[N - 1]);
    oh_fence(Rc[8]);
  }
  if constexpr (MOVE) {
    if (status_b >= 0 || nb < 0) return;
    if (skip_b) {
#pragma unroll
      for (int j = 0; j < N; ++j) {
        const double v = D.q[slot][IDX(t, N, j)];
        D.q_spare[0][SPARE(j)] = v;
        D.q_spare[1][SPARE(j)] = v;
      }
      if (move_G) {
#pragma unroll
        for (int k = 0; k < N; ++k) D.G_spare[SPARE(k)] = D.Gfull[slot][IDX(t, N, k)];
      }
      return;
    }
  } else {
    if (status_b >= 0 || skip_b) return;
  }
  const bool first = first_b != 0;
  if constexpr (MODE != EVAL_ONLY) {
    if (first) {
#pragma unroll
      for (int j = 0; j < N; ++j) q[j] = D.q[slot][IDX(t, N, j)];
      if constexpr (MOVE) {
        if (move_G) {
#pragma unroll
          for (int k = 0; k < N; ++k) D.G_spare[SPARE(k)] = D.Gfull[slot][IDX(t, N, k)];
        }
      }
    } else {
      if constexpr (!OH_RETRACT_PREFETCH) {
#pragma unroll
        for (int a = 0; a < NZ; ++a) zs[a] = D.zstep[IDX(t, NZ, a)];
        load_householder<N>(D.Z[cur], Bp, b, t, Vc);
#pragma unroll
        for (int j = 0; j < N; ++j) q[j] = D.q[cur][IDX(t, N, j)];
#pragma unroll
        for (int i = 0; i < 3 + 3 * NZ; ++i) mdlc[i] = D.mdl[cur][IDX(t, MDL_ROWS(N), i)];
        if constexpr (MOVE) {
          if (move_G) {
#pragma unroll
            for (int k = 0; k < N; ++k) Gmv[k] = D.Gfull[cur][IDX(t, N, k)];
          }
        }
      }
      if constexpr (MOVE) {
#pragma unroll
        for (int j = 0; j < N; ++j) D.q_spare[1][SPARE(j)] = q[j];
        if (move_G) {
#pragma unroll
          for (int k = 0; k < N; ++k) D.G_spare[SPARE(k)] = Gmv[k];
        }
      }
      double Zc[N][NZ];
      z_from_householder<N>(Vc, Zc);
#pragma unroll
      for (int j = 0; j < N; ++j) {
        double v = q[j];
#pragma unroll
        for (int a = 0; a < NZ; ++a) v += Zc[j][a] * zs[a];
        q[j] = asis ? q[j] : v;
      }
#pragma unroll
      for (int m = 0; m < 3; ++m) {
        double v = mdlc[m];
#pragma unroll
        for (int a = 0; a < NZ; ++a) v += mdlc[3 + m * NZ + a] * zs[a];
        e_tgt[m] = v;
      }
    }
  }
  if constexpr (!EARLY) {
#pragma unroll
    for (int i = 0; i < 3; ++i) pc[i] = D.ref[(size_t)i * Bp + b];
#pragma unroll
    for (int i = 0; i < 9; ++i) Rc[i] = D.ref[(size_t)(3 + i) * Bp + b];
  }
  double Gprev[N];
  const bool fresh = first_b == 1;
  bool exact = (P.hessian == OH_HESSIAN_EXACT) || (P.hessian == OH_HESSIAN_HYBRID && !fresh && stat_b <= P.hyb_switch);
  if constexpr (GUARD) {
    if (SPH && GPp->n_links > 0) exact = false;
  }
  const bool have_G = exact && !fresh;
#pragma unroll
  for (int k = 0; k < N; ++k) Gprev[k] = 0.0;

  double phi, cv, g[N], Dr[NP], Z[N][NZ];
  struct Hooks {
    double* __restrict__ qo;
    double* __restrict__ go;
    double* __restrict__ vo;
    const double* __restrict__ Gc;
    int Bp, b, t;
    OH_DEV void q_final(const double (&qv)[N]) const {
      if constexpr (MOVE) {
#pragma unroll
        for (int j = 0; j < N; ++j) qo[SPARE(j)] = qv[j];
        if (qo2) {
#pragma unroll
          for (int j = 0; j < N; ++j) qo2[SPARE(j)] = qv[j];
        }
      } else if constexpr (!GUARD && MODE != EVAL_ONLY) {
#pragma unroll
        for (int j = 0; j < N; ++j) qo[IDX(t, N, j)] = qv[j];
      }
    }
    OH_DEV void g_final(const double (&gv)[N]) const {
      if constexpr (ZC && OH_ZC_EARLY) {
#pragma unroll
        for (int k = 0; k < N; ++k) Go[IDX(t, N, k)] = gv[k] + cpl[k];
      } else if constexpr (ZC) {
        double sm = 0.0;
#pragma unroll
        for (int k = 0; k < N; ++k) {
          const double q0 = qr[k];
          const double dm = q0 - qs[IDX(t - 1, N, k)];
          sm += dm * dm;
          double Gk = gv[k] + kap2 * dm;
          if (!last) Gk -= kap2 * (qs[IDX(t + 1, N, k)] - q0);
          Go[IDX(t, N, k)] = Gk;
        }
        *smo = sm;
      } else if constexpr (!GUARD) {
#pragma unroll
        for (int k = 0; k < N; ++k) go[IDX(t, N, k)] = gv[k];
      }
    }
    OH_DEV void v_final(const double (&Vv)[3][N]) const {
#pragma unroll
      for (int m = 0; m < 3; ++m)
#pragma unroll
        for (int k = m; k < N; ++k) vo[IDX(t, HV_ROWS(N), HV_OFF(N, m) + k - m)] = Vv[m][k];
    }
    const double* Gp;
    OH_DEV void load_G(const double (&)[N], double (&G)[N]) const {
#pragma unroll
      for (int k = 0; k < N; ++k) G[k] = PRE_G ? Gp[k] : Gc[IDX(t, N, k)];
    }
    const double* __restrict__ qs;
    const double* qr;
    double* __restrict__ Go;
    double* smo;
    double kap2;
    bool last;
    const double* cpl;
    double* __restrict__ qo2;
    int nb;
  };
  const Hooks hooks{MOVE ? D.q_spare[0] : D.q[slot], D.g[slot], D.Z[slot], D.Gfull[cur], Bp, b, t, Gpre, D.q[slot], q, D.Gfull[slot], &sm_zc, 2.0 * P.kappa, t == P.T - 1, cpl_zc,
                    (MOVE && first) ? D.q_spare[1] : nullptr, nb};
  double e_new[3], JZ_new[3][NZ];
  const double tol_r = (first_b == 2 || asis) ? 1e300 : retract_tol(P, !first, pred_b, stat_b);
  if constexpr (LEAD)
    eval_knot<N, true, Hooks, MODE>(OH_CHAIN(D), P, t, q, pc, Rc, exact, have_G, Gprev, phi, cv, g, Dr, Z, !first, e_tgt, tol_r, e_new, JZ_new,
                                    D.lead[(size_t)t * Bp + b], hooks);
  else eval_knot<N, false, Hooks, MODE>(OH_CHAIN(D), P, t, q, pc, Rc, exact, have_G, Gprev, phi, cv, g, Dr, Z, !first, e_tgt, tol_r, e_new, JZ_new, 0.0, hooks);
  if constexpr (MODE == EVAL_RETRACT_ONLY) return;
#pragma unroll
  for (int m = 0; m < 3; ++m) {
    D.mdl[slot][IDX(t, MDL_ROWS(N), m)] = e_new[m];
#pragma unroll
    for (int a = 0; a < NZ; ++a) D.mdl[slot][IDX(t, MDL_ROWS(N), 3 + m * NZ + a)] = JZ_new[m][a];
  }
  if constexpr (GUARD) {
    const GuardParams& GP = *GPp;
    const GuardBuffers& GB = *GBp;
    const bool upd = GB.outer[b] != 0;
    const double rho_old = GB.rho[b];
    const double rho = upd ? GB.rho_next[b] : rho_old;
    const double irho = 1.0 / rho, i2rho = 1.0 / (2.0 * rho);
    double psi = 0.0, meas = 0.0, dd[N];
    const int nl = GP.limits ? 2 * N : 0;
#pragma unroll
    for (int j = 0; j < N; ++j) dd[j] = 0.0;
    if (GP.limits) {
#pragma unroll
    for (int j = 0; j < N; ++j) {
#pragma unroll
      for (int side = 0; side < 2; ++side) {
        const double gval = side ? GP.up[j] - q[j] : q[j] - GP.lo[j];
        double* lam_ptr = GB.lam + IDX(t, GP.NC, side * N + j);
        double lam = *lam_ptr;
        if (upd) {
          lam = fmax(0.0, lam - rho_old * gval);
          *lam_ptr = lam;
        }
        const double sv = lam - rho * gval;
        meas = fmax(meas, fabs(fmin(gval, lam * irho)));
        if (sv > 0.0) {
          psi += (sv * sv - lam * lam) * i2rho;
          g[j] += side ? sv : -sv;
          dd[j] += rho;
        } else {
          psi -= lam * lam * i2rho;
        }
      }
    }
    }
#pragma unroll
    for (int a = 0; a < NZ; ++a)
#pragma unroll
      for (int c2 = 0; c2 <= a; ++c2) {
        double acc = 0.0;
#pragma unroll
        for (int j = 0; j < N; ++j) acc += dd[j] * Z[j][a] * Z[j][c2];
        Dr[tri(a, c2)] += acc;
      }
    if (SPH && GP.n_links > 0) {
      sphere_rows_walk<N>(D.chain, GP, GB.par, (size_t)Bp, b, q, [&](const int l, const int o, const double gval, const double (&dg)[N]) {
        double* lam_ptr = GB.lam + IDX(t, GP.NC, nl + l * GP.n_obs + o);
        double lam = *lam_ptr;
        if (upd) {
          lam = fmax(0.0, lam - rho_old * gval);
          *lam_ptr = lam;
        }
        const double sv = lam - rho * gval;
        meas = fmax(meas, fabs(fmin(gval, lam * irho)));
        if (sv > 0.0) {
          psi += (sv * sv - lam * lam) * i2rho;
          double v[NZ];
#pragma unroll
          for (int a = 0; a < NZ; ++a) v[a] = 0.0;
#pragma unroll
          for (int j = 0; j < N; ++j) {
            g[j] -= sv * dg[j];
#pragma unroll
            for (int a = 0; a < NZ; ++a) v[a] += Z[j][a] * dg[j];
          }
#pragma unroll
          for (int a = 0; a < NZ; ++a)
#pragma unroll
            for (int c2 = 0; c2 <= a; ++c2) Dr[tri(a, c2)] += rho * v[a] * v[c2];
        } else {
// ... 133 lines not shown
#ifndef OH_STEP_PREFETCH_BACK
#define OH_STEP_PREFETCH_BACK 1
#endif
#ifndef OH_STEP_PREFETCH_FWD
#define OH_STEP_PREFETCH_FWD 1
#endif
template <class T_>
OH_DEV T_* slot_of(T_* const (&a)[2], const int s) { return s ? a[1] : a[0]; }
struct StepHead { int go; int cur; LMState lm; };
template <int N, bool GUARD = false>
OH_DEV StepHead step_head(const FigParams& P, const FigBuffers& D, const int b, const int ts, const GuardBuffers* GBp, int cur, LMState lm, const int iters) {
  constexpr int NZ = N - 3;
  const int Bp = D.Bp;
  const int T = P.T;
  const unsigned lb = (unsigned)b * 8u;
  const unsigned rowB = (unsigned)Bp * 8u;
  bool polish_request = false;
  bool line_search = false;

  {
    double f = D.fconst[b];
    double feas = 0.0, fpsi = 0.0, meas = 0.0;
    const double* const merit_ts = slot_of(D.merit, ts);
    const double* const cv_ts = slot_of(D.cv, ts);
    const double* psi_ts = nullptr;
    const double* mcv_ts = nullptr;
    if constexpr (GUARD) {
      psi_ts = slot_of(GBp->psi, ts);
      mcv_ts = slot_of(GBp->mcv, ts);
    }
    for (int t = P.t0; t < T; ++t) {
      f += rb_ld(KNOT(merit_ts, t, 1), 0, lb);
      feas = fmax(feas, rb_ld(KNOT(cv_ts, t, 1), 0, lb));
      if constexpr (GUARD) {
        fpsi += rb_ld(KNOT(psi_ts, t, 1), 0, lb);
        meas = fmax(meas, rb_ld(KNOT(mcv_ts, t, 1), 0, lb));
      }
    }
    bool accept;
    if (D.first[b]) {
      if (!(f == f) || !(fabs(f) < 1e300)) {
        D.status[b] = OH_STATUS_NUMERICAL;
        D.cur[b] = ts;
        D.f_cur[b] = f;
        D.stat[b] = f;
        return StepHead{0, cur, lm};
      }
      accept = true;
      D.first[b] = 0;
      if constexpr (GUARD) {
        if (GBp->outer[b]) {
          GBp->outer[b] = 0;
          GBp->rho[b] = GBp->rho_next[b];
        }
      }
    } else if (GUARD && GBp->outer[b]) {
      accept = true;
      GBp->outer[b] = 0;
      GBp->rho[b] = GBp->rho_next[b];
    } else if (D.polish[b]) {
      accept = true;
      D.polish[b] = 0;
    } else {
      const LMState lm_before = lm;
      accept = lm_accept(P, f, feas, D.f_cur[b], D.pred[b], D.stat[b], lm, D.feas[b]);
      polish_request = !accept && !D.stale[b] && D.feas[b] > 10.0 * retract_tol(P, false, D.pred[b], 0.0);
      if (polish_request) lm = lm_before;
      if constexpr (GUARD) {
        if (!accept && !polish_request && GBp->ls_count[b] < OH_LS_MAX && iters < P.max_iter / 2) {
          lm = lm_before;
          line_search = true;
        }
      }
      D.nun[b] = lm.nun;
    }
    if (!accept && D.stale[b]) {
      D.stale[b] = 0;
      D.first[b] = 1;
      D.polish[b] = 0;
      D.mu[b] = lm.mu;
      D.nun[b] = lm.nun;
      D.cur[b] = cur;
      oh_count(D.work + 1);
      return StepHead{1, cur, lm};
    }
    if (accept) {
      D.stale[b] = 0;
      cur = ts;
      D.f_cur[b] = f;
      D.feas[b] = feas;
      if constexpr (GUARD) {
        D.fpsi[b] = fpsi;
        GBp->meas[b] = meas;
        GBp->ls_count[b] = 0;
      }
    }
    D.cur[b] = cur;
    if (!accept) {
      D.skip[b] = 1;
      oh_count(D.work + 1);
    }
  }
  if constexpr (GUARD) {
    if (line_search) {
      if (iters >= P.max_iter) {
        D.status[b] = OH_STATUS_MAX_ITER;
        return StepHead{0, cur, lm};
      }
      for (int t = P.t0; t < T; ++t) {
#pragma unroll
        for (int a = 0; a < NZ; ++a) rb_st(KNOT(D.zstep, t, NZ), RB(a), lb, OH_LS_SHRINK * rb_ld(KNOT(D.zstep, t, NZ), RB(a), lb));
      }
      const int k = GBp->ls_count[b] + 1;
      GBp->ls_count[b] = k;
      double sk = 1.0;
      for (int i = 0; i < k; ++i) sk *= OH_LS_SHRINK;
      D.pred[b] = -sk * GBp->ls_gd[b] + 0.5 * sk * sk * GBp->ls_q[b];
      D.iters[b] = iters + 1;
      return StepHead{1, cur, lm};
    }
  }
  if (polish_request) {
    for (int t = P.t0; t < T; ++t) {
#pragma unroll
      for (int a = 0; a < NZ; ++a) rb_st(KNOT(D.zstep, t, NZ), RB(a), lb, 0.0);
    }
    D.pred[b] = 0.0;
    D.polish[b] = 1;
    D.iters[b] = iters + 1;
    if (iters < P.max_iter + 40) return StepHead{1, cur, lm};
    D.status[b] = OH_STATUS_MAX_ITER;
    return StepHead{0, cur, lm};
  }
  return StepHead{2, cur, lm};
}

template <int N, bool GUARD = false>
OH_DEV bool step_instance(const FigParams& P, const FigBuffers& D, const int b, const int ts, const GuardBuffers* GBp = nullptr) {
  constexpr int NZ = N - 3;
  constexpr int NP = NZ * (NZ + 1) / 2;
  const int Bp = D.Bp;
  const int T = P.T;
  const unsigned lb = (unsigned)b * 8u;
  const unsigned rowB = (unsigned)Bp * 8u;
  const double kap2 = 2.0 * P.kappa;
  int cur = 1 - ts;
  LMState lm{D.mu[b], D.nun[b]};
  const int iters = D.iters[b];
  {
    const StepHead hd = step_head<N, GUARD>(P, D, b, ts, GBp, cur, lm, iters);
    if (hd.go != 2) return hd.go == 1;
    cur = hd.cur;
    lm = hd.lm;
  }
  double mu = lm.mu;

  const double* __restrict__ Ec = D.E[0];
  const double* __restrict__ Drc = D.Dr[0];
  const double* __restrict__ gtc = D.gt[0];
  const unsigned oE = lb + (cur ? (unsigned)((const char*)D.E[1] - (const char*)D.E[0]) : 0u);
  const unsigned oD = lb + (cur ? (unsigned)((const char*)D.Dr[1] - (const char*)D.Dr[0]) : 0u);
  const unsigned oG = lb + (cur ? (unsigned)((const char*)D.gt[1] - (const char*)D.gt[0]) : 0u);
  double stat = 0.0;
  double S[NP], rd[NZ], rn[NZ];
  bool factored = false;
  double quad = 0.0;
// ... 507 lines not shown
```

optas_amd/csrc/oh_handle.h:

```cpp
#pragma once
#include <hip/hip_runtime.h>

#include <array>
#include <map>
#include <string>
#include <vector>

#include "oh_kernels.h"
#include "oh_carve.h"
#include "oh_jit.h"

int fail(int code, const std::string& msg);

#define HIPCHK(expr)                                                                                   \
  do {                                                                                                 \
    hipError_t _e = (expr);                                                                            \
    if (_e != hipSuccess) {                                                                            \
      return fail(OH_ERR_HIP, std::string(#expr) + ": " + hipGetErrorString(_e));                     \
    }                                                                                                  \
  } while (0)

#define OH_PINNED_STAGE_BYTES (256 * 1024)

template <class T, bool PINNED = false>
struct DevBuf {
  T* p = nullptr;
  size_t cap = 0;
  DevBuf() = default;
  DevBuf(const DevBuf&) = delete;
  DevBuf& operator=(const DevBuf&) = delete;
  ~DevBuf() { release(); }
  operator T*() const { return p; }
  void release() {
    if (p) (void)(PINNED ? hipHostFree(p) : hipFree(p));
    p = nullptr;
    cap = 0;
  }
  hipError_t reserve(const size_t n, bool* grew = nullptr) {
    if (grew) *grew = false;
    if (n <= cap) return hipSuccess;
    release();
    const hipError_t e = PINNED ? hipHostMalloc((void**)&p, n * sizeof(T)) : hipMalloc((void**)&p, n * sizeof(T));
    if (e != hipSuccess) {
      p = nullptr;
      return e;
    }
    cap = n;
    if (grew) *grew = true;
    return hipSuccess;
  }
};

struct Solve {
  int B;
  const double *x0, *p;
  double *x, *f, *kkt;
  int *iters, *status;
  Solve part(const size_t lo, const int n, const Shape& sh) const {
    const auto at = [lo](auto* q, const size_t per) -> decltype(q) { return q ? q + lo * per : nullptr; };
    return {n, at(x0, sh.nx), at(p, sh.npar), at(x, sh.nx), at(f, 1), at(kkt, 3), at(iters, 1), at(status, 1)};
  }
};

struct Sched {
  int compaction = 1;
  int compact_carry = 1;
  int compact_fused = 1;
  int tail_vel_threshold = 1 << 30;
  int lg_split = 1;
  int tail_vel = 1;
  int compact_sort = 1;
  double compact_frac = 0.97;
  double compact_frac_restart = 0.9;
  int tail_threshold = 16384;
  int sparse_check_below = 2048;
  int fuse_couple = 1;
  int free_pcr_max = 1536;
  int specialize = OH_SPECIALIZE_AUTO;
  int tq_check = 4;
  std::array<double, 4> inv_saved{1.0, 16384.0, 1.0, -2.0};
};

struct oh_handle;
struct LastSolve {
  struct Part { const oh_handle* q; int n; };
  int B = 0;
  std::vector<Part> parts;
  bool pipe_cache = false;
};


struct TapeState {
  TapeParams P{};
  DevBuf<int> op, a, b, rows;
  DevBuf<double> c;
  DevBuf<double> work;
  DevBuf<double> mult;
  DevBuf<double> h0;
  int cap() const { return (int)(mult.cap / (size_t)(P.n_ineq + P.n_eq + 1)); }
  TapeJit jit;
  TapeJit jit_phi;
  int phi_lds = 0;
  TapeWave wave;
  std::vector<int> h_op, h_a, h_b, h_rows;
  std::vector<double> h_c;
  oh_tape_desc desc{};
};

struct QpState {
  oh_qp_desc desc{};
  DevBuf<double> work;
  DevBuf<double> mult;
  DevBuf<double> blk;
  int last_block = 0;
  bool use_tape = false;
  DevBuf<double> rows, val, f0;
  DevBuf<int> xdep;
  int n_xdep = 0;
};

struct IkState {
  oh_ik_desc desc{};
  DevBuf<double> mult;
};

struct TqState {
  oh_torque_desc desc{};
  TqParams P{};
  TqBuffers D{};
  DevBuf<char> pool;
  DevBuf<double> mult, hc;
};

struct PmState {
  oh_pointmass_desc desc{};
  PmParams P{};
  PmBuffers D{};
  DevBuf<char> pool;
  int cap_B = 0;
};

struct oh_handle {
  oh_problem_desc desc;
  int device = 0;
  hipStream_t stream = nullptr;
  hipEvent_t ev0 = nullptr, ev1 = nullptr, evt0 = nullptr, evt1 = nullptr;
  Sched sch;
  std::map<std::string, double> opt;
  DevBuf<char> stage;
  DevBuf<char, true> h_stage;
  LastSolve last;
  bool profiling = false;
  std::vector<hipEvent_t> prof_events;
  std::vector<int> prof_tags;
  double timing[8] = {0, 0, 0, 0, 0, 0, 0, 0};
  double timing_couple = 0;
  double rejects = 0;
  double tail_iters = 0;
  DevBuf<int, true> h_flag;
  bool have_chain = false;
  oh_chain chain_host;
  DevBuf<oh_chain> d_chain;
  bool have_frames = false;
  OhLinkFrames frames_host;
  DevBuf<OhLinkFrames> d_frames;
  bool have_dyn = false;
  oh_dynamics dyn_host;
  DevBuf<oh_dynamics> d_dyn;
  const FkSpec* fk_spec = nullptr;
  bool fk_spec_failed = false;
  int specialize_min_units = 1 << 16;
  TapeState tape;
  QpState qp;
  IkState ik;
  TqState tq;
  PmState pm;
  std::vector<double> local_path;
  DevBuf<double> d_local_path;
  int cap_B = 0;
  FigBuffers D{};
  FigParams P{};
  DevBuf<char> pool;
  bool have_guards = false;
  oh_guards guards{};
  GuardParams GP{};
  GuardBuffers GB{};
  DevBuf<char> gpool;
  int gcap = 0;
  DevBuf<char> move_scr;
  int free_sweep_last = -1;
  int free_sweeps_used = 0;
  int specialize_min_B = 4096;
  const FigSpec* spec = nullptr;
  bool spec_failed = false;
  bool spec_move_failed = false;
  bool spec_cache_checked = false;
  double spec_seconds = 0.0;
  std::vector<oh_handle*> peers;
  DevBuf<double> d_pipe_mult;
  bool is_peer = false;
  ~oh_handle() {
    for (oh_handle* p : peers) delete p;
    hipSetDevice(device);
    if (stream) hipStreamSynchronize(stream);
    for (hipEvent_t e : prof_events) hipEventDestroy(e);
    for (hipEvent_t e : {ev0, ev1, evt0, evt1})
      if (e) hipEventDestroy(e);
    oh_tape_jit_release(&tape.jit);
    oh_tape_jit_release(&tape.jit_phi);
    oh_tape_wave_release(&tape.wave);
    if (stream) hipStreamDestroy(stream);
  }
};

struct OptDoc { const char* name; double dflt; };
static constexpr OptDoc OPT_TABLE[] = {
    {"check_every", 1},        {"row_pad", 13},          {"retract_min", 1e-13}, {"hyb_switch", 1e-5},   {"relax", 1.5},          {"relax_from", 4},         {"settle_k", 1.0},   {"al_fuse", 1},   {"streams", 2},         {"split_min", 65536},  {"tq_split_min", 1024}, {"free_split_min", 256},
    {"free_bb", 1},            {"free_persist", -1},     {"free_cp_max", 512},   {"pm_wave_max", 20480}, {"qp_mode", -1},         {"tape_lds_max", 1 << 30},
    {"tape_wave", 1},          {"tape_lbfgs", -1},       {"tape_wave_nt", 256},  {"tape_wave_regs", -1}, {"tape_wave_hist", -1},  {"tq_stall", 25},
    {"tq_curv_after", 3},      {"tq_ftb", 0.995},        {"tq_theta_mu", 1.35},  {"tq_kappa_mu", 0.4},   {"tq_curv_from", 0.1},   {"tq_jac_dual", 0},
    {"tq_rebuild", 0.9},         {"compact_move_all", 1},  {"tq_curv_late", 1.0},  {"tq_kappa_eps", 10.0}, {"tq_max_back", 3},     {"tq_mu_dec", 1.0 / 3.0},     {"tq_ls_curv", 1},   {"tq_mu_dec_warm", 0.1}, {"tq_curv_lag", 3},
    {"tol", 0},                {"pipe", 1},               {"pipe_chunk", 32768},                {"invariant_compact_frac", 0.65}, {"invariant_split", 1}, {"invariant_move_slim", 1}, {"invariant_move_live", 1},
};
constexpr int opt_row(const char* name) {
  for (int i = 0; i < (int)(sizeof(OPT_TABLE) / sizeof(OPT_TABLE[0])); ++i) {
    int k = 0;
    while (OPT_TABLE[i].name[k] && OPT_TABLE[i].name[k] == name[k]) ++k;
    if (OPT_TABLE[i].name[k] == name[k]) return i;
  }
  return -1;
}
template <int ROW>
constexpr int known_opt() {
  static_assert(ROW >= 0, "optv: the option is not in OPT_TABLE");
  return ROW;
}
inline double opt_value(const oh_handle* h, const OptDoc& d) {
  const auto it = h->opt.find(d.name);
  return it == h->opt.end() ? d.dflt : it->second;
}
#define optv(h, name) opt_value(h, OPT_TABLE[known_opt<opt_row(name)>()])
inline double batch_invariant(const oh_handle* h) {
  const auto it = h->opt.find("batch_invariant");
  return it == h->opt.end() ? 0.0 : it->second;
}

enum { OPEN_CHAIN = 1, OPEN_FLAG = 2 };
oh_handle* open_handle(const std::string& who, int kind, int T, int ndof, int want, int* rc);
void reset_counters(oh_handle* h);
int finish_solve(oh_handle* h, double launched);
Shape shape_of(const oh_handle* h);
bool solver_chain_ok(const oh_chain& c);
int validate_chain(const oh_handle* h, const oh_chain& c);
void adopt_chain(oh_handle* h, const oh_chain& c);
void drop_peers(oh_handle* h);
int ensure_stage(oh_handle* h, size_t bytes);
template <class Layout>
int stage_carve(oh_handle* h, Layout&& layout) {
  if (const int rc = ensure_stage(h, layout(Carver(nullptr, Carver::Slots)))) return rc;
  layout(Carver(h->stage.p, Carver::Slots));
  return OH_OK;
}

int tape_solve_device(oh_handle* h, const Solve& a);
int qp_solve_device(oh_handle* h, const Solve& a);
int ik_solve_device(oh_handle* h, const Solve& a);
int pm_solve_device(oh_handle* h, const Solve& a);
int tq_solve_device(oh_handle* h, const Solve& a, double mu_b0_warm = 0.0);
int tape_validate(const oh_tape_desc* d, const char* who);
TapeParams tape_params(const oh_tape_desc* d, int lbfgs_opt = -1);
int tape_configure(oh_handle* h);
int upload_tape(oh_handle* h, const oh_tape_desc* d, const int* op_override);
size_t qp_np(const oh_qp_desc& q);
int specialize_fk(oh_handle* h);
```

optas_amd/csrc/oh_kernels.h:

```cpp
#pragma once
#include <hip/hip_runtime.h>

#include <string>
#include <vector>

#include "optas_hip.h"
#include "oh_types.h"

struct OhKernelInfo {
  int vgprs, scratch_bytes, lds_bytes, block, blocks_per_cu;
};
bool oh_kernel_info_figure8(const char* name, OhKernelInfo* out);
bool oh_kernel_info_fkjac(const char* name, OhKernelInfo* out);
bool oh_kernel_info_torque(const char* name, OhKernelInfo* out);
bool oh_kernel_info_linkkin(const char* name, OhKernelInfo* out);
bool oh_kernel_info_qp_block(const char* name, OhKernelInfo* out);

void oh_launch_fk_jac(hipStream_t s, bool soa, const oh_chain* d_chain, int n_chain, int ndof, int n, const double* q, double* pose, double* J);
struct OhLinkFrames {
  oh_chain link, base;
  int n_shared;
};
void oh_launch_link_kin(hipStream_t s, bool soa, const OhLinkFrames* d_frames, int n_link, int n, const double* q, const double* a3, const oh_link_out& out);
bool oh_launch_setup(hipStream_t s, int n, const FigParams& P, const FigBuffers& D, const double* x0, const double* p);
bool oh_launch_eval(hipStream_t s, int n, const FigParams& P, const FigBuffers& D, int slot, int part = 0);
bool oh_launch_carry(hipStream_t s, int n, const FigParams& P, const FigBuffers& D, int phase, int Bnew, int slot);
bool oh_launch_eval_lead(hipStream_t s, int n, const FigParams& P, const FigBuffers& D, int slot);
bool oh_launch_couple(hipStream_t s, int n, const FigParams& P, const FigBuffers& D, int slot);
bool oh_launch_couple_vel(hipStream_t s, int n, const FigParams& P, const FigBuffers& D, const GuardParams& GP, const GuardBuffers& GB, int slot);
bool oh_launch_step(hipStream_t s, int n, const FigParams& P, const FigBuffers& D, int slot);
bool oh_launch_eval_free(hipStream_t s, int n, const FigParams& P, const FigBuffers& D, int slot);
bool oh_launch_couple_free(hipStream_t s, int n, const FigParams& P, const FigBuffers& D, int slot);
bool oh_launch_couple_free_vel(hipStream_t s, int n, const FigParams& P, const FigBuffers& D, const GuardParams& GP, const GuardBuffers& GB, int slot);
enum FreeSweep { FREE_SERIAL, FREE_PCR, FREE_CP, FREE_BB, FREE_PERSIST };
bool oh_launch_step_free(hipStream_t s, int n, const FigParams& P, const FigBuffers& D, int slot, FreeSweep sweep);
void oh_launch_move_rows(hipStream_t s, void* arr, void* scr, int rows, int Bp, int B, int Bnew, const int* newidx, bool is_int);
void oh_launch_move_rows_live(hipStream_t s, double* a0, double* a1, double* scr, int rows, int Bp, int B, int Bnew, const int* newidx, const int* cur, const int* curn);
bool oh_launch_setup_guards(hipStream_t s, int n, const FigParams& P, const FigBuffers& D, const GuardParams& GP, const GuardBuffers& GB, const double* p);
void oh_launch_guard_infeasible(hipStream_t s, int n, const FigParams& P, const FigBuffers& D, const GuardParams& GP, const double* p, int B, double* kkt, int* status);
bool oh_launch_eval_guarded(hipStream_t s, int n, const FigParams& P, const FigBuffers& D, const GuardParams& GP, const GuardBuffers& GB, int slot);
bool oh_launch_free_persist(hipStream_t s, int n, const FigParams& P, const FigBuffers& D, const GuardParams& GP, const GuardBuffers& GB);
bool oh_launch_step_guarded(hipStream_t s, int n, const FigParams& P, const FigBuffers& D, const GuardParams& GP, const GuardBuffers& GB, int slot,
                            FreeSweep sweep);
bool oh_launch_eval_locked_guarded(hipStream_t s, int n, const FigParams& P, const FigBuffers& D, const GuardParams& GP, const GuardBuffers& GB, int slot, int part);
bool oh_launch_step_locked_guarded(hipStream_t s, int n, const FigParams& P, const FigBuffers& D, const GuardParams& GP, const GuardBuffers& GB, int slot);
void oh_launch_guard_emit(hipStream_t s, const FigParams& P, const FigBuffers& D, const GuardParams& GP, const GuardBuffers& GB, int NV, int only_done);
void oh_launch_guard_compact(hipStream_t s, const FigParams& P, const FigBuffers& D, const GuardParams& GP, const GuardBuffers& GB, int NV, int phase, int Bnew);
bool oh_launch_tail(hipStream_t s, int n, const FigParams& P, const FigBuffers& D, int slot);
bool oh_launch_tail_vel(hipStream_t s, int n, const FigParams& P, const FigBuffers& D, const GuardParams& GP, const GuardBuffers& GB, int slot);
bool oh_launch_finalize(hipStream_t s, int n, const FigParams& P, const FigBuffers& D, int only_done, double* x, double* f, double* kkt,
                        int* iters, int* status, int parts = 3);
void oh_launch_scan_running(hipStream_t s, const FigBuffers& D, int sort);
bool oh_launch_compact(hipStream_t s, int n, const FigParams& P, const FigBuffers& D, int phase, int Bnew, int slot);

struct PmParams {
  int T;
  double dt, w_acc, ylim, vlim, safe_sq, tol;
  int max_iter;
  int final_only;
  double w_vel;
  int fix_vf;
};
struct PmBuffers {
  int B, Bp;
  double *a, *X, *s, *lam, *K, *kk, *dX, *da;
};
void oh_launch_pm_solve(hipStream_t s, const PmParams& P, const PmBuffers& D, const double* x0, const double* p, double* x, double* f, double* kkt,
                        int* iters, int* status, int wave_max);

void oh_launch_pm_tick_params(hipStream_t s, int B, int T, int tick, int advance, double ramp, const double* state, const double* obs_table, double* p);
void oh_launch_pm_advance(hipStream_t s, int B, int T, int advance, const double* x, double* state_next);

#define TQ_XS 24
#define TQ_SD 448
#define TQ_SD_GB 272
#define TQ_SD_J 296
#define TQ_LAM 32
#define TQ_HC 232
#define TQ_GN 128
struct TqParams {
  int T, N, max_iter;
  double dt, w_path, w_vel, w_tau, tol, tol_compl, mu_b0, mu0;
  double theta;
  double mu_dec;
  double kappa_eps, kappa_mu, theta_mu;
  double curv_from;
  double curv_late;
  int curv_after;
  int stall_max;
  double tau_ftb;
  int max_back;
  int curv_lag;
  int ls_curv;
  double tau_lo[OH_MAX_CHAIN], tau_up[OH_MAX_CHAIN];
  double dq_lo[OH_MAX_CHAIN], dq_up[OH_MAX_CHAIN];
  int vel;
  int jac_closed_form;
  int nx, np;
};
struct TqBuffers {
  int B;
  const oh_chain* chain;
  const oh_dynamics* dyn;
  double* xs;
  double* st;
  double* lam;
  double* gains;
  double* goal;
  double* hc;
  double *f_cur, *f_true, *bsum, *mu, *nun, *mub, *stat, *alpha, *qk, *ndx, *viol;
  int* curv_age;
  int *cur, *first, *curv, *status, *iters, *rejected, *n_barrier, *nrel, *n_back, *stall;
  int* n_running;
// ... 87 lines not shown
```

optas_amd/csrc/oh_kernels.hip:

```cpp
#include "oh_platform_gfx950.h"
#include "oh_figure8_kernels.h"
#include "oh_kernels.h"

#define OH_DISPATCH_N(n, call)         \
  switch (n) {                         \
    case 4: call(4); break;            \
    case 5: call(5); break;            \
    case 6: call(6); break;            \
    case 7: call(7); break;            \
    case 8: call(8); break;            \
    default: return false;             \
  }
#define OH_DISPATCH_N_ANY(n, call)     \
  switch (n) {                         \
    case 2: call(2); break;            \
    case 3: call(3); break;            \
    case 4: call(4); break;            \
    case 5: call(5); break;            \
    case 6: call(6); break;            \
    case 7: call(7); break;            \
    case 8: call(8); break;            \
    default: return false;             \
  }

// ... 58 lines not shown
  const bool running = alive && !skipping;
  {
    const unsigned long long m = __ballot(running);
    if ((threadIdx.x & 63) == 0 && m) atomicAdd(D.work, (unsigned long long)__popcll(m));
  }
  bool still = skipping;
  if (skipping) D.skip[b] = 0;
  if (running) still = step_instance<N, true>(P, D, b, slot, &GB);
  const unsigned long long m2 = __ballot(still);
  if ((threadIdx.x & 63) == 0 && m2) atomicAdd(D.n_running, __popcll(m2));
}
bool oh_launch_eval_locked_guarded(hipStream_t s, int n, const FigParams& P, const FigBuffers& D, const GuardParams& GP, const GuardBuffers& GB, int slot, int part) {
  const dim3 g((D.B + 255) / 256, P.T - P.t0), b(256);
#define C(NN)                                                                              \
  if (part == 0) hipLaunchKernelGGL(k_eval_lg<NN>, g, b, 0, s, P, D, GP, GB, slot);       \
  else if (part == 1) hipLaunchKernelGGL(k_retract<NN>, g, b, 0, s, P, D, slot);          \
  else hipLaunchKernelGGL(k_evalb_lg<NN>, g, b, 0, s, P, D, GP, GB, slot)
  OH_DISPATCH_N(n, C)
#undef C
  return true;
}
bool oh_launch_step_locked_guarded(hipStream_t s, int n, const FigParams& P, const FigBuffers& D, const GuardParams& GP, const GuardBuffers& GB, int slot) {
  const dim3 g((D.B + 63) / 64), b(64);
#define C(NN) hipLaunchKernelGGL(k_step_lg<NN>, g, b, 0, s, P, D, GB, slot)
  OH_DISPATCH_N(n, C)
#undef C
  return true;
}
#ifndef OH_STEP_WAVES
#define OH_STEP_WAVES 2
#endif
template <int N>
__global__ __launch_bounds__(64, OH_STEP_WAVES) void k_step(FigParams P, FigBuffers D, const int slot) {
  const int b = blockIdx.x * blockDim.x + threadIdx.x;
  const bool alive = (b < D.B) && (D.status[b] < 0);
  const bool skipping = alive && D.skip[b];
  const bool running = alive && !skipping;
  {
    const unsigned long long m = __ballot(running);
    if ((threadIdx.x & 63) == 0 && m) atomicAdd(D.work, (unsigned long long)__popcll(m));
  }
  bool still = skipping;
  if (skipping) D.skip[b] = 0;
  if (running) still = step_instance<N>(P, D, b, slot);
  const unsigned long long m2 = __ballot(still);
  if ((threadIdx.x & 63) == 0 && m2) atomicAdd(D.n_running, __popcll(m2));
}

#ifndef OH_STEP_ZC_WAVES
#define OH_STEP_ZC_WAVES 1
#endif
template <int N>
__global__ __launch_bounds__(64, OH_STEP_ZC_WAVES) void k_step_zc(FigParams P, FigBuffers D, const int slot) {
  __shared__ double zl[N * (N - 3)][64];
  const int b = blockIdx.x * blockDim.x + threadIdx.x;
  const bool alive = (b < D.B) && (D.status[b] < 0);
  const bool skipping = alive && D.skip[b];
  const bool running = alive && !skipping;
  {
    const unsigned long long m = __ballot(running);
    if ((threadIdx.x & 63) == 0 && m) atomicAdd(D.work, (unsigned long long)__popcll(m));
  }
  bool still = skipping;
  if (skipping) D.skip[b] = 0;
  if (running) still = step_instance_zc<N>(P, D, b, slot, &zl[0][threadIdx.x]);
  const unsigned long long m2 = __ballot(still);
  if ((threadIdx.x & 63) == 0 && m2) atomicAdd(D.n_running, __popcll(m2));
}

template <int N>
__global__ __launch_bounds__(256) void k_defer_copy(FigParams P, FigBuffers D, const int slot) {
  const int n = D.n_defer[slot];
  if (blockIdx.x == 0 && threadIdx.x == 0) D.n_defer[1 - slot] = 0;
  const int Bp = D.Bp, nk = P.T - P.t0;
  const long long total = (long long)n * nk;
  for (long long i = (long long)blockIdx.x * blockDim.x + threadIdx.x; i < total; i += (long long)gridDim.x * blockDim.x) {
    const int e = (int)(i / nk), t = P.t0 + (int)(i % nk);
    const int b = D.defer_list[(size_t)slot * Bp + e];
    const int cur = D.cur[b];
    const double* __restrict__ Gold = D.Gfull[1 - cur];
    double* __restrict__ Gnew = D.Gfull[cur];
#pragma unroll
    for (int k = 0; k < N; ++k) Gnew[IDX(t, N, k)] = Gold[IDX(t, N, k)];
  }
}

template <int N>
__global__ __launch_bounds__(64) void k_tail(FigParams P, FigBuffers D, const int slot) { tail_block<N>(P, D, slot); }
template <int N>
__global__ __launch_bounds__(64) void k_tail_vel(FigParams P, FigBuffers D, GuardParams GP, GuardBuffers GB, const int slot) {
  tail_block<N, true>(P, D, slot, &GP, &GB);
}

template <int N>
__global__ __launch_bounds__(256) void k_finalize(FigParams P, FigBuffers D, int only_done, double* __restrict__ x, double* __restrict__ f,
                                                  double* __restrict__ kkt, int* __restrict__ iters, int* __restrict__ status) {
  finalize_unit<N>(P, D, only_done, x, f, kkt, iters, status, blockIdx.x * blockDim.x + threadIdx.x, blockIdx.y);
}
constexpr int SCAN_NB = 8;
constexpr int SCAN_TPB = 256;
constexpr int SCAN_MAXBLK = 1024;
OH_DEV int scan_class(const FigBuffers& D, const int b, const int sort) {
  if (!sort) return 0;
  int e = 0;
  frexp(D.stat[b], &e);
  const int k = (e + 24) / 4;
  return k < 0 ? 0 : (k > SCAN_NB - 1 ? SCAN_NB - 1 : k);
}
OH_DEV void scan_block(const FigBuffers& D, const int sort, const int chunk, int (&c)[SCAN_NB], int (*cnt)[SCAN_TPB], int& lo, int& hi) {
  const int tid = threadIdx.x;
  const int per = (chunk + SCAN_TPB - 1) / SCAN_TPB;
  const int blo = blockIdx.x * chunk;
  lo = blo + tid * per;
  hi = min(min(D.B, blo + chunk), lo + per);
#pragma unroll
  for (int k = 0; k < SCAN_NB; ++k) c[k] = 0;
  for (int b = lo; b < hi; ++b)
    if (D.status[b] < 0) {
      const int kb = scan_class(D, b, sort);
#pragma unroll
      for (int k = 0; k < SCAN_NB; ++k) c[k] += (k == kb);
    }
#pragma unroll
  for (int k = 0; k < SCAN_NB; ++k) cnt[k][tid] = c[k];
  __syncthreads();
  for (int off = 1; off < SCAN_TPB; off <<= 1) {
    int v[SCAN_NB];
#pragma unroll
    for (int k = 0; k < SCAN_NB; ++k) v[k] = (tid >= off) ? cnt[k][tid - off] : 0;
    __syncthreads();
#pragma unroll
    for (int k = 0; k < SCAN_NB; ++k) cnt[k][tid] += v[k];
    __syncthreads();
  }
}
__global__ __launch_bounds__(SCAN_TPB) void k_scan_count(FigBuffers D, const int sort, const int chunk, int* __restrict__ blk) {
  __shared__ int cnt[SCAN_NB][SCAN_TPB];
  int c[SCAN_NB], lo, hi;
  scan_block(D, sort, chunk, c, cnt, lo, hi);
  if (threadIdx.x < SCAN_NB) blk[threadIdx.x * SCAN_MAXBLK + blockIdx.x] = cnt[threadIdx.x][SCAN_TPB - 1];
}
__global__ __launch_bounds__(SCAN_MAXBLK) void k_scan_offsets(FigBuffers D, const int nblk, int* __restrict__ blk) {
  __shared__ int sc[SCAN_MAXBLK];
  __shared__ int carry;
  const int tid = threadIdx.x;
  if (tid == 0) carry = 0;
  __syncthreads();
  for (int k = 0; k < SCAN_NB; ++k) {
    const int mine = (tid < nblk) ? blk[k * SCAN_MAXBLK + tid] : 0;
    sc[tid] = mine;
    __syncthreads();
    for (int off = 1; off < SCAN_MAXBLK; off <<= 1) {
      const int v = (tid >= off) ? sc[tid - off] : 0;
      __syncthreads();
      sc[tid] += v;
      __syncthreads();
    }
    if (tid < nblk) blk[k * SCAN_MAXBLK + tid] = carry + sc[tid] - mine;
    __syncthreads();
    if (tid == 0) carry += sc[SCAN_MAXBLK - 1];
    __syncthreads();
  }
  if (tid == 0) *D.n_new = carry;
}
__global__ __launch_bounds__(SCAN_TPB) void k_scan_assign(FigBuffers D, const int sort, const int chunk, const int* __restrict__ blk) {
  __shared__ int cnt[SCAN_NB][SCAN_TPB];
  int c[SCAN_NB], lo, hi;
  scan_block(D, sort, chunk, c, cnt, lo, hi);
  int pos[SCAN_NB];
#pragma unroll
  for (int k = 0; k < SCAN_NB; ++k) pos[k] = blk[k * SCAN_MAXBLK + blockIdx.x] + cnt[k][threadIdx.x] - c[k];
  for (int b = lo; b < hi; ++b) {
    if (D.status[b] < 0) {
      const int kb = scan_class(D, b, sort);
      int p = 0;
#pragma unroll
      for (int k = 0; k < SCAN_NB; ++k)
        if (k == kb) p = pos[k]++;
      D.newidx[b] = p;
    } else {
      D.newidx[b] = -1;
    }
  }
}

template <int N>
__global__ __launch_bounds__(256) void k_compact_gather(FigParams P, FigBuffers D) {
  const int b = blockIdx.x * blockDim.x + threadIdx.x;
  const int t = blockIdx.y;
  const int Bp = D.Bp;
  if (b >= D.B) return;
  const int nb = D.newidx[b];
  if (nb < 0) return;
  const double* __restrict__ qs = D.q[D.cur[b]];
  double* __restrict__ tq = D.Z[1];
  double* __restrict__ ts = D.Dr[1];
#pragma unroll
  for (int j = 0; j < N; ++j) tq[((size_t)t * N + j) * Bp + nb] = qs[IDX(t, N, j)];
  if (P.hessian != OH_HESSIAN_GAUSS_NEWTON || P.zc) {
#pragma unroll
    for (int j = 0; j < N; ++j) D.g[1][((size_t)t * N + j) * Bp + nb] = D.Gfull[D.cur[b]][IDX(t, N, j)];
  }
  if (t == 0) {
#pragma unroll
    for (int i = 0; i < 12; ++i) ts[(size_t)i * Bp + nb] = D.ref[(size_t)i * Bp + b];
    ts[(size_t)12 * Bp + nb] = D.fconst[b];
    ts[(size_t)13 * Bp + nb] = D.mu[b];
    ts[(size_t)14 * Bp + nb] = (double)(D.iters[b] + (D.polish[b] == 2 ? 1 : 0));
    ts[(size_t)15 * Bp + nb] = (double)D.orig[b];
    ts[(size_t)16 * Bp + nb] = D.nun[b];
    ts[(size_t)17 * Bp + nb] = D.stat[b];
  }
}
template <int N>
__global__ __launch_bounds__(256) void k_compact_scatter(FigParams P, FigBuffers D, int Bnew, const int slot) {
  const int b = blockIdx.x * blockDim.x + threadIdx.x;
  const int t = blockIdx.y;
  const int Bp = D.Bp;
  if (b >= Bnew) return;
  const double* __restrict__ tq = D.Z[1];
  const double* __restrict__ ts = D.Dr[1];
#pragma unroll
  for (int j = 0; j < N; ++j) {
    const double v = tq[IDX(t, N, j)];
    D.q[slot][IDX(t, N, j)] = v;
    if (t < P.t0) D.q[1 - slot][IDX(t, N, j)] = v;
    if (P.hessian != OH_HESSIAN_GAUSS_NEWTON || P.zc) D.Gfull[1 - slot][IDX(t, N, j)] = D.g[1][IDX(t, N, j)];
  }
  if (t == 0) {
#pragma unroll
    for (int i = 0; i < 12; ++i) D.ref[(size_t)i * Bp + b] = ts[(size_t)i * Bp + b];
    D.fconst[b] = ts[(size_t)12 * Bp + b];
    D.mu[b] = ts[(size_t)13 * Bp + b];
    D.nun[b] = ts[(size_t)16 * Bp + b];
    const int it = (int)ts[(size_t)14 * Bp + b];
    D.iters[b] = it > 0 ? it - 1 : 0;
    D.orig[b] = (int)ts[(size_t)15 * Bp + b];
    D.cur[b] = 1 - slot;
    D.stat[b] = ts[(size_t)17 * Bp + b];
    D.first[b] = 2;
    D.skip[b] = 0;
    D.polish[b] = 0;
    D.stale[b] = 0;
    D.status[b] = -1;
  }
}

template <int N, bool REST = false>
__global__ __launch_bounds__(256) void k_carry_gather(FigParams P, FigBuffers D, const int slot) {
  const int b = blockIdx.x * blockDim.x + threadIdx.x;
  const int t = blockIdx.y;
  const int Bp = D.Bp;
  if (b >= D.B) return;
  const int nb = D.newidx[b];
  if (nb < 0) return;
  const bool restart = D.skip[b] != 0 || D.first[b] != 0;
  const int cur = restart ? slot : 1 - slot;
  double* __restrict__ t_trial = D.q_spare[0];
  double* __restrict__ t_cur = D.q_spare[1];
  double* __restrict__ t_G = D.G_spare;
  double* __restrict__ ts = D.Dr[1];
  if (!REST || t < P.t0) {
#pragma unroll
    for (int j = 0; j < N; ++j) {
      t_trial[((size_t)t * N + j) * Bp + nb] = D.q[slot][IDX(t, N, j)];
      t_cur[((size_t)t * N + j) * Bp + nb] = D.q[cur][IDX(t, N, j)];
      if (P.hessian != OH_HESSIAN_GAUSS_NEWTON || P.zc) t_G[((size_t)t * N + j) * Bp + nb] = D.Gfull[cur][IDX(t, N, j)];
    }
  }
  if (t == 0) {
#pragma unroll
    for (int i = 0; i < 12; ++i) ts[(size_t)i * Bp + nb] = D.ref[(size_t)i * Bp + b];
    ts[(size_t)12 * Bp + nb] = D.fconst[b];
    ts[(size_t)13 * Bp + nb] = D.mu[b];
    ts[(size_t)14 * Bp + nb] = (double)(D.iters[b] - ((D.skip[b] != 0 && D.first[b] == 0) ? 1 : 0));
    ts[(size_t)15 * Bp + nb] = (double)D.orig[b];
    ts[(size_t)16 * Bp + nb] = D.nun[b];
    ts[(size_t)17 * Bp + nb] = D.f_cur[b];
    ts[(size_t)18 * Bp + nb] = D.pred[b];
    ts[(size_t)19 * Bp + nb] = D.stat[b];
    ts[(size_t)20 * Bp + nb] = D.feas[b];
    ts[(size_t)21 * Bp + nb] = (double)((restart ? 1 : 0) + 2 * (D.polish[b] != 0 ? 1 : 0) + 4 * (D.polish[b] == 2 ? 1 : 0));
  }
}
template <int N>
__global__ __launch_bounds__(256) void k_carry_scatter(FigParams P, FigBuffers D, int Bnew, const int slot) {
  const int b = blockIdx.x * blockDim.x + threadIdx.x;
  const int Bp = D.Bp;
  if (b >= Bnew) return;
  const double* __restrict__ ts = D.Dr[1];
  {
#pragma unroll
    for (int i = 0; i < 12; ++i) D.ref[(size_t)i * Bp + b] = ts[(size_t)i * Bp + b];
    const int flags = (int)ts[(size_t)21 * Bp + b];
    const bool restart = (flags & 1) != 0;
    D.fconst[b] = ts[(size_t)12 * Bp + b];
    D.mu[b] = ts[(size_t)13 * Bp + b];
    const int it = (int)ts[(size_t)14 * Bp + b];
    D.iters[b] = it > 0 ? it : 0;
    D.orig[b] = (int)ts[(size_t)15 * Bp + b];
    D.nun[b] = ts[(size_t)16 * Bp + b];
    D.f_cur[b] = ts[(size_t)17 * Bp + b];
    D.pred[b] = ts[(size_t)18 * Bp + b];
    D.stat[b] = ts[(size_t)19 * Bp + b];
    D.feas[b] = ts[(size_t)20 * Bp + b];
    D.cur[b] = 1 - slot;
    D.first[b] = restart ? 1 : 0;
    D.skip[b] = 0;
    D.polish[b] = (!restart && (flags & 2)) ? ((flags & 4) ? 2 : 1) : 0;
    D.stale[b] = restart ? 0 : 1;
    D.status[b] = -1;
  }
}

template <int N>
static void launch_setup_t(hipStream_t s, const FigParams& P, const FigBuffers& D, const double* x0, const double* p) {
  hipLaunchKernelGGL(k_setup<N>, dim3((D.B + 63) / 64, P.T), dim3(64), 0, s, P, D, x0, p);
}
template <int N>
static void launch_eval_t(hipStream_t s, const FigParams& P, const FigBuffers& D, int slot, int part) {
  const dim3 ge((D.B + 255) / 256, P.T - P.t0);
  if (part != 2) hipLaunchKernelGGL(k_retract<N>, ge, dim3(256), 0, s, P, D, slot);
  if (part != 1) {
    if (P.zc) hipLaunchKernelGGL(k_evalb_zc<N>, dim3((((D.B + 255) / 256) + 7) / 8 * 8 * (P.T - P.t0)), dim3(256), 0, s, P, D, slot);
    else hipLaunchKernelGGL(k_evalb<N>, ge, dim3(256), 0, s, P, D, slot);
  }
}
template <int N>
static void launch_carry_t(hipStream_t s, const FigParams& P, const FigBuffers& D, int phase, int Bnew, int slot) {
  if (phase == 0) hipLaunchKernelGGL(k_carry_gather<N>, dim3((D.B + 255) / 256, P.T), dim3(256), 0, s, P, D, slot);
  else if (phase == 2) hipLaunchKernelGGL((k_carry_gather<N, true>), dim3((D.B + 255) / 256, P.t0 > 1 ? P.t0 : 1), dim3(256), 0, s, P, D, slot);
  else hipLaunchKernelGGL(k_carry_scatter<N>, dim3((Bnew + 255) / 256), dim3(256), 0, s, P, D, Bnew, slot);
}
template <int N>
static void launch_couple_t(hipStream_t s, const FigParams& P, const FigBuffers& D, int slot) {
  const int nbx8 = (((D.B + 255) / 256) + 7) / 8 * 8;
  hipLaunchKernelGGL(k_couple<N>, dim3(nbx8 * (P.T - P.t0)), dim3(256), 0, s, P, D, slot);
}
template <int N>
static void launch_step_t(hipStream_t s, const FigParams& P, const FigBuffers& D, int slot) {
  if (P.zc) {
    hipLaunchKernelGGL(k_step_zc<N>, dim3((D.B + 63) / 64), dim3(64), 0, s, P, D, slot);
    if (P.hessian != OH_HESSIAN_GAUSS_NEWTON) hipLaunchKernelGGL(k_defer_copy<N>, dim3(512), dim3(256), 0, s, P, D, slot);
  } else hipLaunchKernelGGL(k_step<N>, dim3((D.B + 63) / 64), dim3(64), 0, s, P, D, slot);
}
template <int N>
static void launch_tail_t(hipStream_t s, const FigParams& P, const FigBuffers& D, int slot) {
  hipLaunchKernelGGL(k_tail<N>, dim3(D.B), dim3(64), 0, s, P, D, slot);
}
template <int N>
__global__ __launch_bounds__(256) void k_finalize_x(FigParams P, FigBuffers D, const int only_done, double* __restrict__ x) {
  constexpr int TK = 8, ROWS = (TK + 1) * N;
  __shared__ double tile[ROWS][65];
  __shared__ long long orig_s[64];
  const int Bp = D.Bp;
  const int lane = threadIdx.x & 63, w = threadIdx.x >> 6;
  const int b = blockIdx.x * 64 + lane, t0 = blockIdx.y * TK;
  bool emit = b < D.B;
  if (emit && only_done && D.status[b] < 0) emit = false;
  if (w == 0) orig_s[lane] = emit ? (long long)D.orig[b] : -1;
  const int nk = min(TK + 1, P.T - t0);
  if (emit) {
    const double* __restrict__ qs = D.q[D.cur[b]];
    for (int row = w; row < nk * N; row += 4) tile[row][lane] = qs[IDX(t0 + row / N, N, row % N)];
  }
  __syncthreads();
  const int nq = min(TK, P.T - t0) * N, ndq = min(TK, P.T - 1 - t0) * N;
  const double inv_dt = 1.0 / P.dt;
  for (int i = w; i < 64; i += 4) {
    const long long ob = orig_s[i];
    if (ob < 0) continue;
    double* xb = x + (size_t)ob * P.nx;
    if (lane < nq) xb[(size_t)t0 * N + lane] = tile[lane][i];
    if (lane < ndq) xb[(size_t)P.T * N + (size_t)t0 * N + lane] = (tile[lane + N][i] - tile[lane][i]) * inv_dt;
  }
}
template <int N>
static void launch_finalize_t(hipStream_t s, const FigParams& P, const FigBuffers& D, int only_done, double* x, double* f, double* kkt,
                              int* iters, int* status, const int parts) {
  if (x && (parts & 1)) hipLaunchKernelGGL(k_finalize_x<N>, dim3((D.B + 63) / 64, (P.T + 7) / 8), dim3(256), 0, s, P, D, only_done, x);
  if (!(parts & 2)) return;
  hipLaunchKernelGGL(k_finalize<N>, dim3((D.B + 255) / 256, D.lam_h ? P.T : 1), dim3(256), 0, s, P, D, only_done, (double*)nullptr, f, kkt, iters, status);
}
template <int N>
static void launch_compact_t(hipStream_t s, const FigParams& P, const FigBuffers& D, int phase, int Bnew, int slot) {
  if (phase == 0) hipLaunchKernelGGL(k_compact_gather<N>, dim3((D.B + 255) / 256, P.T), dim3(256), 0, s, P, D);
  else hipLaunchKernelGGL(k_compact_scatter<N>, dim3((Bnew + 255) / 256, P.T), dim3(256), 0, s, P, D, Bnew, slot);
}

bool oh_launch_setup(hipStream_t s, int n, const FigParams& P, const FigBuffers& D, const double* x0, const double* p) {
#define C(NN) launch_setup_t<NN>(s, P, D, x0, p)
  OH_DISPATCH_N_ANY(n, C)
#undef C
  return true;
}
bool oh_launch_eval(hipStream_t s, int n, const FigParams& P, const FigBuffers& D, int slot, int part) {
#define C(NN) launch_eval_t<NN>(s, P, D, slot, part)
  OH_DISPATCH_N(n, C)
#undef C
  return true;
}
bool oh_launch_carry(hipStream_t s, int n, const FigParams& P, const FigBuffers& D, int phase, int Bnew, int slot) {
#define C(NN) launch_carry_t<NN>(s, P, D, phase, Bnew, slot)
  OH_DISPATCH_N(n, C)
#undef C
  return true;
}
bool oh_launch_couple(hipStream_t s, int n, const FigParams& P, const FigBuffers& D, int slot) {
#define C(NN) launch_couple_t<NN>(s, P, D, slot)
  OH_DISPATCH_N(n, C)
#undef C
  return true;
}
bool oh_launch_couple_vel(hipStream_t s, int n, const FigParams& P, const FigBuffers& D, const GuardParams& GP, const GuardBuffers& GB, int slot) {
  const int Tn = P.T - P.t0;
  const dim3 gu((D.B + 255) / 256, Tn), gc((unsigned)(((D.B + 255) / 256 + 7) / 8 * 8 * Tn)), b(256);
#define C(NN)                                                              \
  hipLaunchKernelGGL(k_vel_update<NN>, gu, b, 0, s, P, D, GP, GB, slot);  \
  hipLaunchKernelGGL(k_couple_vel<NN>, gc, b, 0, s, P, D, GP, GB, slot)
  OH_DISPATCH_N(n, C)
#undef C
  return true;
}
bool oh_launch_step(hipStream_t s, int n, const FigParams& P, const FigBuffers& D, int slot) {
#define C(NN) launch_step_t<NN>(s, P, D, slot)
  OH_DISPATCH_N(n, C)
#undef C
  return true;
}
bool oh_launch_tail_vel(hipStream_t s, int n, const FigParams& P, const FigBuffers& D, const GuardParams& GP, const GuardBuffers& GB, int slot) {
#define C(NN) hipLaunchKernelGGL(k_tail_vel<NN>, dim3(D.B), dim3(64), 0, s, P, D, GP, GB, slot)
  OH_DISPATCH_N(n, C)
#undef C
  return true;
}
bool oh_launch_tail(hipStream_t s, int n, const FigParams& P, const FigBuffers& D, int slot) {
#define C(NN) launch_tail_t<NN>(s, P, D, slot)
  OH_DISPATCH_N(n, C)
#undef C
  return true;
}
bool oh_launch_finalize(hipStream_t s, int n, const FigParams& P, const FigBuffers& D, int only_done, double* x, double* f, double* kkt,
                        int* iters, int* status, int parts) {
#define C(NN) launch_finalize_t<NN>(s, P, D, only_done, x, f, kkt, iters, status, parts)
  OH_DISPATCH_N_ANY(n, C)
#undef C
  return true;
}
void oh_launch_scan_running(hipStream_t s, const FigBuffers& D, int sort) {
  int nblk = (D.B + 1023) / 1024;
  if (nblk > SCAN_MAXBLK) nblk = SCAN_MAXBLK;
  if (nblk < 1) nblk = 1;
  const int chunk = (D.B + nblk - 1) / nblk;
  hipLaunchKernelGGL(k_scan_count, dim3(nblk), dim3(SCAN_TPB), 0, s, D, sort, chunk, D.scan_blk);
  hipLaunchKernelGGL(k_scan_offsets, dim3(1), dim3(SCAN_MAXBLK), 0, s, D, nblk, D.scan_blk);
  hipLaunchKernelGGL(k_scan_assign, dim3(nblk), dim3(SCAN_TPB), 0, s, D, sort, chunk, D.scan_blk);
}
template <class V>
__global__ __launch_bounds__(256) void k_move_gather(const V* __restrict__ src, V* __restrict__ scr, const int Bp, const int B, const int* __restrict__ newidx) {
  const int b = blockIdx.x * blockDim.x + threadIdx.x;
  if (b >= B) return;
  const int nb = newidx[b];
  if (nb < 0) return;
  const size_t row = (size_t)blockIdx.y * Bp;
  scr[row + nb] = src[row + b];
}
template <class V>
__global__ __launch_bounds__(256) void k_move_scatter(V* __restrict__ dst, const V* __restrict__ scr, const int Bp, const int Bnew) {
  const int b = blockIdx.x * blockDim.x + threadIdx.x;
  if (b >= Bnew) return;
  const size_t row = (size_t)blockIdx.y * Bp;
  dst[row + b] = scr[row + b];
}
__global__ __launch_bounds__(256) void k_move_gather_live(const double* __restrict__ src0, const double* __restrict__ src1, double* __restrict__ scr, const int Bp,
                                                          const int B, const int* __restrict__ newidx, const int* __restrict__ cur) {
  const int b = blockIdx.x * blockDim.x + threadIdx.x;
  if (b >= B) return;
  const int nb = newidx[b];
  if (nb < 0) return;
  const size_t row = (size_t)blockIdx.y * Bp;
  scr[row + nb] = (cur[b] ? src1 : src0)[row + b];
}
__global__ __launch_bounds__(256) void k_move_scatter_live(double* __restrict__ dst0, double* __restrict__ dst1, const double* __restrict__ scr, const int Bp,
                                                           const int Bnew, const int* __restrict__ curn) {
  const int b = blockIdx.x * blockDim.x + threadIdx.x;
  if (b >= Bnew) return;
  const size_t row = (size_t)blockIdx.y * Bp;
  (curn[b] ? dst1 : dst0)[row + b] = scr[row + b];
}
void oh_launch_move_rows_live(hipStream_t s, double* a0, double* a1, double* scr, int rows, int Bp, int B, int Bnew, const int* newidx, const int* cur, const int* curn) {
  if (!a0 || !a1 || rows <= 0) return;
  const dim3 gg((B + 255) / 256, rows), gs((Bnew + 255) / 256, rows), blk(256);
  hipLaunchKernelGGL(k_move_gather_live, gg, blk, 0, s, (const double*)a0, (const double*)a1, scr, Bp, B, newidx, cur);
  hipLaunchKernelGGL(k_move_scatter_live, gs, blk, 0, s, a0, a1, (const double*)scr, Bp, Bnew, curn);
}
void oh_launch_move_rows(hipStream_t s, void* arr, void* scr, int rows, int Bp, int B, int Bnew, const int* newidx, bool is_int) {
  if (!arr || rows <= 0) return;
  const dim3 gg((B + 255) / 256, rows), gs((Bnew + 255) / 256, rows), blk(256);
  if (is_int) {
    hipLaunchKernelGGL(k_move_gather<int>, gg, blk, 0, s, (const int*)arr, (int*)scr, Bp, B, newidx);
    hipLaunchKernelGGL(k_move_scatter<int>, gs, blk, 0, s, (int*)arr, (const int*)scr, Bp, Bnew);
  } else {
    hipLaunchKernelGGL(k_move_gather<double>, gg, blk, 0, s, (const double*)arr, (double*)scr, Bp, B, newidx);
    hipLaunchKernelGGL(k_move_scatter<double>, gs, blk, 0, s, (double*)arr, (const double*)scr, Bp, Bnew);
  }
}

bool oh_launch_compact(hipStream_t s, int n, const FigParams& P, const FigBuffers& D, int phase, int Bnew, int slot) {
// ... 30 lines not shown
```

optas_amd/csrc/oh_types.h:

```cpp
#pragma once
#include "optas_hip.h"

struct FigParams {
  int T;
  int t0;
  int lock;
  int path_in_frame;
  int nx;
  double dt;
  double w_path;
  double kappa;
  double tol;
  double tol_feas;
  double tol_retract;
  double tol_retract_min;
  double feas_accept;
  int max_retract;
  int max_iter;
  int hessian;
  double hyb_switch;
  double mu0;
  double relax;
  int relax_from;
  int al_fuse;
// ... 3 lines not shown
  int zc;
  int zc_free;
  int inst_major;
};

struct GuardParams {
  int limits, n_links, n_obs, NC;
  int link_joint[OH_MAX_SPHERE_LINKS];
  double link_off[OH_MAX_SPHERE_LINKS][3];
  double lo[OH_MAX_CHAIN], up[OH_MAX_CHAIN];
  double rho0;
  int vel;
  double vlo[OH_MAX_CHAIN], vup[OH_MAX_CHAIN];
  double vscale;
};
struct GuardBuffers {
  double* lam;
  double* par;
  double* psi[2];
  double* rho;
  double* rho_next;
  double* omega;
  double* meas_prev;
  int* outer;
  int* n_outer;
  double* mcv[2];
  double* meas;
  double* lamv;
  double* lam_out;
  double* lamv_out;
  double* scr;
  int* ls_count;
  double* ls_gd;
  double* ls_q;
};
#define OH_LS_MAX 3
#define OH_LS_SHRINK 0.3

struct FigBuffers {
  int B, Bp;
  const oh_chain* chain;
  double* q[2];
  double* q_spare[2];
  double* G_spare;
  double* Z[2];
  double* Dr[2];
  double* g[2];
  double* phi[2];
  double* cv[2];
  double* Gfull[2];
  double* mdl[2];
  double* E[2];
  double* gt[2];
  double* merit[2];
  double* zstep;
  double* Kmat;
  double* kvec;
  double* ref;
  double* fconst;
  double* f_cur;
  double* pred;
  double* mu;
  double* nun;
  double* stat;
  double* feas;
  double* fpsi;
  double* lead;
  int* cur;
  int* first;
  int* scan_blk;
  int* skip;
  int* polish;
  int* stale;
  int* status;
  int* iters;
  int* orig;
  int* newidx;
  int* n_running;
  int* n_new;
  double* lam_h;
  unsigned long long* work;
  int* n_defer;
  int* defer_list;
};
```

Measured before the change: 3.157 million solves/s.

## Add lean compaction mode that skips redundant q/G copies and rescues rejected lanes

Adds a 'lean' carry-compaction mode, now on by default through compact_fused=2. During compaction it stops writing the backup q_spare[1] copy and moves G only for hybrid lanes that need it. Rejected steps are recorded in a rescue list and repaired afterwards by a new sweep kernel, which also absorbs the deferred G copy formerly done by k_defer_copy. This cuts memory traffic during compaction, at the cost of a wider host readback of list counts and an extra sweep launch on every iteration.

```diff
diff --git a/include/optas_hip.h b/include/optas_hip.h
--- a/include/optas_hip.h
+++ b/include/optas_hip.h
@@ -270,7 +270,7 @@
 int oh_link_kin_device(oh_handle* h, int N, const void* d_q, const double* axis3, const oh_link_out* d_out_soa);
 
 int oh_set_profiling(oh_handle* h, int enable);
-int oh_get_timing(oh_handle* h, double* out11);
+int oh_get_timing(oh_handle* h, double* out14);
 
 enum { OH_SPECIALIZE_NEVER = 0, OH_SPECIALIZE_ALWAYS = 1, OH_SPECIALIZE_AUTO = 2 };
 int oh_specialize(oh_handle* h);
diff --git a/optas_amd/backend.py b/optas_amd/backend.py
--- a/optas_amd/backend.py
+++ b/optas_amd/backend.py
@@ -70,7 +70,7 @@
         )
 
     def solve_ms(self) -> float:
-        out = (C.c_double * 11)()
+        out = (C.c_double * 14)()
         _lib.check(_lib.load().oh_get_timing(self._h, out), "oh_get_timing")
         return out[4]
 
@@ -453,7 +453,7 @@
         return states, tau0, f, iters, status
 
     def timing(self) -> dict:
-        out = (C.c_double * 11)()
+        out = (C.c_double * 14)()
         _lib.check(_lib.load().oh_get_timing(self._h, out), "oh_get_timing")
         return {"solve_ms": out[4], "iterations_launched": int(out[5]), "work_instances": out[6], "eval_ms": out[0], "step_ms": out[2]}
 
@@ -611,7 +611,7 @@
         ch = getattr(self, "_chunked", None)
         if ch is not None:
             return dict(ch["timing"])
-        out = (C.c_double * 11)()
+        out = (C.c_double * 14)()
         _lib.check(_lib.load().oh_get_timing(self._h, out), "oh_get_timing")
         return {
             "eval_ms": out[0],
@@ -625,6 +625,9 @@
             "couple_ms": out[8],
             "rejected_steps": int(out[9]),
             "tail_iterations": int(out[10]),
+            "rescued_instances": int(out[11]),
+            "gradient_lanes_moved": int(out[12]),
+            "lanes_moved": int(out[13]),
         }
 
     def fk_jac_soa_device(self, n: int, d_q, d_pose, d_J) -> None:
diff --git a/optas_amd/csrc/oh_api.hip b/optas_amd/csrc/oh_api.hip
--- a/optas_amd/csrc/oh_api.hip
+++ b/optas_amd/csrc/oh_api.hip
@@ -35,7 +35,7 @@
 static const FieldOpt FIELD_OPTS[] = {
     {"tail_threshold", &Sched::tail_threshold}, {"free_pcr_max", &Sched::free_pcr_max}, {"compaction", &Sched::compaction, nullptr, true},
     {"compact_frac", nullptr, &Sched::compact_frac}, {"compact_sort", &Sched::compact_sort}, {"compact_carry", &Sched::compact_carry},
-    {"compact_fused", &Sched::compact_fused, nullptr, true},
+    {"compact_fused", &Sched::compact_fused},
     {"tail_vel", &Sched::tail_vel}, {"lg_split", &Sched::lg_split}, {"tail_vel_threshold", &Sched::tail_vel_threshold},
     {"fuse_couple", &Sched::fuse_couple, nullptr, true}, {"sparse_check_below", &Sched::sparse_check_below}, {"specialize", &Sched::specialize},
     {"tq_check", &Sched::tq_check},
@@ -135,7 +135,7 @@
   bool ok = hipStreamCreate(&h->stream) == hipSuccess;
   for (hipEvent_t* e : {&h->ev0, &h->ev1, &h->evt0, &h->evt1}) ok = ok && hipEventCreate(e) == hipSuccess;
   if ((want & OPEN_CHAIN) && ok) ok = h->d_chain.reserve(1) == hipSuccess;
-  if ((want & OPEN_FLAG) && ok) ok = h->h_flag.reserve(1) == hipSuccess;
+  if ((want & OPEN_FLAG) && ok) ok = h->h_flag.reserve(16) == hipSuccess;
   if (!ok) {
     delete h;
     *rc = fail(OH_ERR_HIP, who + (want ? ": stream/event/allocation failed" : ": stream/event creation failed"));
@@ -146,7 +146,7 @@
 
 void reset_counters(oh_handle* h) {
   for (double& t : h->timing) t = 0.0;
-  h->timing_couple = h->rejects = h->tail_iters = 0.0;
+  h->timing_couple = h->rejects = h->tail_iters = h->rescued = h->grad_moved = h->lanes_moved = 0.0;
 }
 int finish_solve(oh_handle* h, const double launched) {
   HIPCHK(hipEventRecord(h->ev1, h->stream));
@@ -549,7 +549,7 @@
 }
 static int solve_device(oh_handle* h, const Solve& a, bool may_fan_out, LastSolve* rec);
 struct Tally {
-  double launched = 0, work = 0, compactions = 0, rejects = 0, tails = 0;
+  double launched = 0, work = 0, compactions = 0, rejects = 0, tails = 0, rescued = 0, grad_moved = 0, lanes_moved = 0;
 };
 static int lane_solve(oh_handle* q, Tally& t, const Solve& a) {
   if (const int rc = solve_device(q, a, false, nullptr)) return rc;
@@ -558,6 +558,7 @@
   t.compactions += q->timing[7];
   t.rejects += q->rejects;
   t.tails += q->tail_iters;
+  t.rescued += q->rescued; t.grad_moved += q->grad_moved; t.lanes_moved += q->lanes_moved;
   return OH_OK;
 }
 template <class Work>
@@ -596,6 +597,7 @@
     h->timing[7] += t.compactions;
     h->rejects += t.rejects;
     h->tail_iters += t.tails;
+    h->rescued += t.rescued; h->grad_moved += t.grad_moved; h->lanes_moved += t.lanes_moved;
   }
   return OH_OK;
 }
@@ -623,6 +625,7 @@
   double *x, *f, *kkt;
   int *iters, *status;
   int launched, compactions;
+  double lanes_moved;
   size_t ne;
 };
 static FreeSweep free_sweep(oh_handle* h, const int nb, const bool start = false) {
@@ -649,13 +652,22 @@
 static bool check_after(const oh_handle* h, const Traj& r, const int it, const bool tail_ok) {
   return (it + 1) % ((!tail_ok && r.check_every == 1 && h->D.B <= h->sch.sparse_check_below) ? 8 : r.check_every) == 0;
 }
-static int look(oh_handle* h, const bool check, int* nrun) {
+struct ListCounts { int defer[2], rescue; };
+static int look(oh_handle* h, const bool check, int* nrun, ListCounts* lists = nullptr) {
   *nrun = -1;
   if (!check) return OH_OK;
   hipStream_t s = h->stream;
-  HIPCHK(hipMemcpyAsync(h->h_flag, h->D.n_running, sizeof(int), hipMemcpyDeviceToHost, s));
+  const FigBuffers& D = h->D;
+  const size_t span = (size_t)((const char*)(D.n_rescue + 1) - (const char*)D.n_running);
+  const bool wide = lists && (const char*)D.n_defer > (const char*)D.n_running && span <= 16 * sizeof(int);
+  HIPCHK(hipMemcpyAsync(h->h_flag, D.n_running, wide ? span : sizeof(int), hipMemcpyDeviceToHost, s));
+  if (lists && !wide) HIPCHK(hipMemcpyAsync(h->h_flag.p + 1, D.n_defer, 3 * sizeof(int), hipMemcpyDeviceToHost, s));
   HIPCHK(hipStreamSynchronize(s));
   *nrun = *h->h_flag;
+  if (lists) {
+    const int* c = wide ? h->h_flag.p + (D.n_defer - D.n_running) : h->h_flag.p + 1;
+    *lists = ListCounts{{c[0], c[1]}, c[2]};
+  }
   return OH_OK;
 }
 static void finalize(oh_handle* h, const Traj& r, const int only_done) {
@@ -717,7 +729,7 @@
     }
   }
   HIPCHK(hipEventRecord(h->ev0, s));
-  HIPCHK(hipMemsetAsync(h->D.work, 0, 4 * sizeof(unsigned long long), s));
+  HIPCHK(hipMemsetAsync(h->D.work, 0, 7 * sizeof(unsigned long long), s));
   if (!oh_launch_setup(s, r.N, h->P, h->D, x0, r.p)) return fail(OH_ERR_INVALID, "oh_solve_device: unsupported ndof");
   if (r.guarded) oh_launch_setup_guards(s, r.N, h->P, h->D, h->GP, h->GB, r.p);
   h->prof_tags.clear();
@@ -751,6 +763,10 @@
   const bool carry = h->sch.compaction && h->sch.compact_carry && (size_t)h->desc.T * ((N - 3) * (N - 2) / 2) >= 22 && !r.guarded && !r.lead;
   const double inv_frac = optv(h, "invariant_compact_frac");
   const bool inv_move = r.invariant && !r.lead && inv_frac > 0.0, restart = h->sch.compaction && !r.lead, restart_moves = r.guarded && optv(h, "compact_move_all") != 0.0;
+  const bool lean = carry && r.spec && r.spec->retract_move && h->sch.compact_fused >= 2 && P.zc && P.hessian != OH_HESSIAN_GAUSS_NEWTON && !r.invariant;
+  D.lean = 0;
+  if (lean) HIPCHK(h->h_flag.reserve(16));
+  int rescue_slot = -1;
   int nrun = -1, carry_pending = 0;
   for (int it = 0; it < r.hard_cap; ++it) {
     if (nrun >= 0)
@@ -765,6 +781,7 @@
       bool moved = false, scanned = false;
       if (r.spec && r.spec->retract_move && h->sch.compact_fused && !h->spec_move_failed) {
         finalize(h, r, 1);
+        D.lean = lean ? (optv(h, "lean_count") != 0.0 ? 3 : 1) : 0;
         oh_launch_scan_running(s, D, h->sch.compact_sort);
         scanned = true;
         if (const int rc = mark(h, r, 0)) return rc;
@@ -772,9 +789,14 @@
         if (moved) {
           if (const int rc = mark(h, r, 4)) return rc;
           oh_launch_carry(s, N, P, D, 2, 0, slot);
+          if (lean) {
+            rescue_slot = slot;
+            r.lanes_moved += carry_pending;
+          }
         } else {
           (void)hipGetLastError();
           h->spec_move_failed = true;
+          D.lean = 0;
         }
       }
       if (!moved) {
@@ -788,7 +810,7 @@
       }
       oh_launch_carry(s, N, P, D, 1, carry_pending, slot);
       std::swap(D.q[slot], D.q_spare[0]);
-      std::swap(D.q[1 - slot], D.q_spare[1]);
+      if (rescue_slot < 0) std::swap(D.q[1 - slot], D.q_spare[1]);
       if (P.hessian != OH_HESSIAN_GAUSS_NEWTON || P.zc) std::swap(D.Gfull[1 - slot], D.G_spare);
       D.B = carry_pending;
       carry_pending = 0;
@@ -802,10 +824,20 @@
     const bool check = check_after(h, r, it, tail_ok);
     if (const int rc = mark(h, r, 3)) return rc;
     if (r.guarded) oh_launch_step_locked_guarded(s, N, P, D, GP, GB, slot);
-    else oh_launch_step(s, N, P, D, slot);
+    else oh_launch_step(s, N, P, D, slot, !lean);
     if (const int rc = mark(h, r, 2)) return rc;
     ++r.launched;
-    if (const int rc = look(h, check, &nrun)) return rc;
+    ListCounts lists{{0, 0}, 0};
+    if (const int rc = look(h, check, &nrun, lean ? &lists : nullptr)) return rc;
+    if (lean) {
+      const bool rescue = rescue_slot >= 0;
+      if (!check || lists.defer[0] || lists.defer[1] || (rescue && lists.rescue))
+        oh_launch_sweep_lists(s, N, P, D, slot, rescue, check ? std::max(lists.defer[slot], rescue ? lists.rescue : 0) : -1);
+      if (rescue) {
+        std::swap(D.q[1 - rescue_slot], D.q_spare[1]);
+        rescue_slot = -1;
+      }
+    }
     if (nrun == 0) break;
     if (tail_ok && nrun > 0 && nrun <= tail_threshold) {
       if (const int rc = compact_batch(h, r, nrun, (it + 1) & 1, false)) return rc;
@@ -873,12 +905,13 @@
   h->D.B = r.B;
   if (r.guarded) oh_launch_guard_infeasible(s, r.N, h->P, h->D, h->GP, r.p, r.B, r.kkt, r.status);
   if (const int frc = finish_solve(h, r.launched)) return frc;
-  unsigned long long work[3] = {0, 0, 0};
+  unsigned long long work[7] = {0, 0, 0, 0, 0, 0, 0};
   HIPCHK(hipMemcpyAsync(work, h->D.work, sizeof(work), hipMemcpyDeviceToHost, s));
   HIPCHK(hipStreamSynchronize(s));
   h->timing[6] = (double)work[0];
   h->rejects = (double)work[1];
   h->tail_iters = (double)work[2];
+  h->rescued = (double)work[5]; h->grad_moved = (double)work[6]; h->lanes_moved = r.lanes_moved;
   if (r.prof) {
     double ms[4] = {0, 0, 0, 0};
     int n[5] = {0, 0, 0, 0, 0};
@@ -1109,6 +1142,9 @@
   out8[8] = h->timing_couple;
   out8[9] = h->rejects;
   out8[10] = h->tail_iters;
+  out8[11] = h->rescued;
+  out8[12] = h->grad_moved;
+  out8[13] = h->lanes_moved;
   return OH_OK;
 }
 extern "C" int oh_event_timer_start(oh_handle* h) {
diff --git a/optas_amd/csrc/oh_carve.h b/optas_amd/csrc/oh_carve.h
--- a/optas_amd/csrc/oh_carve.h
+++ b/optas_amd/csrc/oh_carve.h
@@ -60,6 +60,8 @@
   D.feas = c.take<double>(Bp);
   D.lam_h = c.take<double>((size_t)4 * T * Bp);
   D.lead = c.take<double>(per_t);
+  D.oldidx = D.lead ? (int*)D.lead : nullptr;
+  D.rescue_list = D.lead ? (int*)D.lead + Bp : nullptr;
   if (!lock) D.lam_h = nullptr;
   D.cur = c.take<int>(Bp);
   D.first = c.take<int>(Bp);
@@ -74,6 +76,7 @@
   D.n_new = c.take<int>(1);
   D.work = c.take<unsigned long long>(14);
   D.n_defer = D.work ? (int*)(D.work + 3) : nullptr;
+  D.n_rescue = D.work ? (int*)(D.work + 4) : nullptr;
   D.scan_blk = c.take<int>(8 * 1024);
   D.defer_list = c.take<int>(2 * (size_t)Bp);
   c.take<int>(2);
diff --git a/optas_amd/csrc/oh_figure8_units.h b/optas_amd/csrc/oh_figure8_units.h
--- a/optas_amd/csrc/oh_figure8_units.h
+++ b/optas_amd/csrc/oh_figure8_units.h
@@ -100,7 +100,9 @@
   const double stat_b = D.stat[b], pred_b = D.pred[b];
   int nb = 0;
   if constexpr (MOVE) nb = D.newidx[b];
-  const bool move_G = MOVE && (P.hessian != OH_HESSIAN_GAUSS_NEWTON || P.zc);
+  const bool lean = MOVE && D.lean != 0;
+  bool move_G = MOVE && (P.hessian != OH_HESSIAN_GAUSS_NEWTON || P.zc);
+  if (lean && P.hessian == OH_HESSIAN_HYBRID) move_G = !skip_b && first_b == 0 && stat_b <= P.hyb_switch;
   double Gmv[N];
   constexpr bool EARLY = MODE == EVAL_ONLY || OH_RETRACT_PREFETCH;
   double Rc[9], pc[3];
@@ -172,7 +174,7 @@
       for (int j = 0; j < N; ++j) {
         const double v = D.q[slot][IDX(t, N, j)];
         D.q_spare[0][SPARE(j)] = v;
-        D.q_spare[1][SPARE(j)] = v;
+        if (!lean) D.q_spare[1][SPARE(j)] = v;
       }
       if (move_G) {
 #pragma unroll
@@ -211,8 +213,10 @@
         }
       }
       if constexpr (MOVE) {
-#pragma unroll
-        for (int j = 0; j < N; ++j) D.q_spare[1][SPARE(j)] = q[j];
+        if (!lean) {
+#pragma unroll
+          for (int j = 0; j < N; ++j) D.q_spare[1][SPARE(j)] = q[j];
+        }
         if (move_G) {
 #pragma unroll
           for (int k = 0; k < N; ++k) D.G_spare[SPARE(k)] = Gmv[k];
@@ -315,7 +319,7 @@
     int nb;
   };
   const Hooks hooks{MOVE ? D.q_spare[0] : D.q[slot], D.g[slot], D.Z[slot], D.Gfull[cur], Bp, b, t, Gpre, D.q[slot], q, D.Gfull[slot], &sm_zc, 2.0 * P.kappa, t == P.T - 1, cpl_zc,
-                    (MOVE && first) ? D.q_spare[1] : nullptr, nb};
+                    (MOVE && first && !lean) ? D.q_spare[1] : nullptr, nb};
   double e_new[3], JZ_new[3][NZ];
   const double tol_r = (first_b == 2 || asis) ? 1e300 : retract_tol(P, !first, pred_b, stat_b);
   if constexpr (LEAD)
@@ -615,6 +619,10 @@
       D.nun[b] = lm.nun;
       D.cur[b] = cur;
       oh_count(D.work + 1);
+      if (D.lean) {
+        D.rescue_list[oh_take_ticket(D.n_rescue)] = b;
+        oh_count(D.work + 5);
+      }
       return StepHead{1, cur, lm};
     }
     if (accept) {
diff --git a/optas_amd/csrc/oh_handle.h b/optas_amd/csrc/oh_handle.h
--- a/optas_amd/csrc/oh_handle.h
+++ b/optas_amd/csrc/oh_handle.h
@@ -65,7 +65,7 @@
 struct Sched {
   int compaction = 1;
   int compact_carry = 1;
-  int compact_fused = 1;
+  int compact_fused = 2;
   int tail_vel_threshold = 1 << 30;
   int lg_split = 1;
   int tail_vel = 1;
@@ -157,6 +157,7 @@
   double timing_couple = 0;
   double rejects = 0;
   double tail_iters = 0;
+  double rescued = 0, grad_moved = 0, lanes_moved = 0;
   DevBuf<int, true> h_flag;
   bool have_chain = false;
   oh_chain chain_host;
@@ -215,7 +216,7 @@
 
 struct OptDoc { const char* name; double dflt; };
 static constexpr OptDoc OPT_TABLE[] = {
-    {"check_every", 1},        {"row_pad", 13},          {"retract_min", 1e-13}, {"hyb_switch", 1e-5},   {"relax", 1.5},          {"relax_from", 4},         {"settle_k", 1.0},   {"al_fuse", 1},   {"streams", 2},         {"split_min", 65536},  {"tq_split_min", 1024}, {"free_split_min", 256},
+    {"check_every", 1},        {"lean_count", 0},        {"row_pad", 13},          {"retract_min", 1e-13}, {"hyb_switch", 1e-5},   {"relax", 1.5},          {"relax_from", 4},         {"settle_k", 1.0},   {"al_fuse", 1},   {"streams", 2},         {"split_min", 65536},  {"tq_split_min", 1024}, {"free_split_min", 256},
     {"free_bb", 1},            {"free_persist", -1},     {"free_cp_max", 512},   {"pm_wave_max", 20480}, {"qp_mode", -1},         {"tape_lds_max", 1 << 30},
     {"tape_wave", 1},          {"tape_lbfgs", -1},       {"tape_wave_nt", 256},  {"tape_wave_regs", -1}, {"tape_wave_hist", -1},  {"tq_stall", 25},
     {"tq_curv_after", 3},      {"tq_ftb", 0.995},        {"tq_theta_mu", 1.35},  {"tq_kappa_mu", 0.4},   {"tq_curv_from", 0.1},   {"tq_jac_dual", 0},
diff --git a/optas_amd/csrc/oh_kernels.h b/optas_amd/csrc/oh_kernels.h
--- a/optas_amd/csrc/oh_kernels.h
+++ b/optas_amd/csrc/oh_kernels.h
@@ -28,7 +28,8 @@
 bool oh_launch_eval_lead(hipStream_t s, int n, const FigParams& P, const FigBuffers& D, int slot);
 bool oh_launch_couple(hipStream_t s, int n, const FigParams& P, const FigBuffers& D, int slot);
 bool oh_launch_couple_vel(hipStream_t s, int n, const FigParams& P, const FigBuffers& D, const GuardParams& GP, const GuardBuffers& GB, int slot);
-bool oh_launch_step(hipStream_t s, int n, const FigParams& P, const FigBuffers& D, int slot);
+bool oh_launch_step(hipStream_t s, int n, const FigParams& P, const FigBuffers& D, int slot, bool with_copy = true);
+bool oh_launch_sweep_lists(hipStream_t s, int n, const FigParams& P, const FigBuffers& D, int slot, bool rescue, int count);
 bool oh_launch_eval_free(hipStream_t s, int n, const FigParams& P, const FigBuffers& D, int slot);
 bool oh_launch_couple_free(hipStream_t s, int n, const FigParams& P, const FigBuffers& D, int slot);
 bool oh_launch_couple_free_vel(hipStream_t s, int n, const FigParams& P, const FigBuffers& D, const GuardParams& GP, const GuardBuffers& GB, int slot);
diff --git a/optas_amd/csrc/oh_kernels.hip b/optas_amd/csrc/oh_kernels.hip
--- a/optas_amd/csrc/oh_kernels.hip
+++ b/optas_amd/csrc/oh_kernels.hip
@@ -164,6 +164,38 @@
     double* __restrict__ Gnew = D.Gfull[cur];
 #pragma unroll
     for (int k = 0; k < N; ++k) Gnew[IDX(t, N, k)] = Gold[IDX(t, N, k)];
+  }
+}
+
+template <int N>
+__global__ __launch_bounds__(256) void k_sweep_lists(FigParams P, FigBuffers D, const int slot, const int rescue) {
+  const int Bp = D.Bp, nk = P.T - P.t0;
+  {
+    const int n = min(D.n_defer[slot], D.B);
+    if (blockIdx.x == 0 && threadIdx.x == 0) D.n_defer[1 - slot] = 0;
+    const long long total = (long long)n * nk;
+    for (long long i = (long long)blockIdx.x * blockDim.x + threadIdx.x; i < total; i += (long long)gridDim.x * blockDim.x) {
+      const int e = (int)(i / nk), t = P.t0 + (int)(i % nk);
+      const int b = D.defer_list[(size_t)slot * Bp + e];
+      const int cur = D.cur[b];
+      const double* __restrict__ Gold = D.Gfull[1 - cur];
+      double* __restrict__ Gnew = D.Gfull[cur];
+#pragma unroll
+      for (int k = 0; k < N; ++k) Gnew[IDX(t, N, k)] = Gold[IDX(t, N, k)];
+    }
+  }
+  if (rescue) {
+    const int n = min(*D.n_rescue, D.B);
+    const long long total = (long long)n * nk;
+    const double* __restrict__ src = D.q[1 - slot];
+    double* __restrict__ dst = D.q_spare[1];
+    for (long long i = (long long)blockIdx.x * blockDim.x + threadIdx.x; i < total; i += (long long)gridDim.x * blockDim.x) {
+      const int e = (int)(i / nk), t = P.t0 + (int)(i % nk);
+      const int b = D.rescue_list[e];
+      const int ob = D.oldidx[b];
+#pragma unroll
+      for (int k = 0; k < N; ++k) dst[IDX(t, N, k)] = src[((size_t)t * N + k) * Bp + ob];
+    }
   }
 }
 
@@ -244,6 +276,7 @@
     __syncthreads();
   }
   if (tid == 0) *D.n_new = carry;
+  if (tid == 0 && D.lean) *D.n_rescue = 0;
 }
 __global__ __launch_bounds__(SCAN_TPB) void k_scan_assign(FigBuffers D, const int sort, const int chunk, const int* __restrict__ blk) {
   __shared__ int cnt[SCAN_NB][SCAN_TPB];
@@ -260,6 +293,7 @@
       for (int k = 0; k < SCAN_NB; ++k)
         if (k == kb) p = pos[k]++;
       D.newidx[b] = p;
+      if (D.lean) D.oldidx[p] = b;
     } else {
       D.newidx[b] = -1;
     }
@@ -363,6 +397,11 @@
     ts[(size_t)19 * Bp + nb] = D.stat[b];
     ts[(size_t)20 * Bp + nb] = D.feas[b];
     ts[(size_t)21 * Bp + nb] = (double)((restart ? 1 : 0) + 2 * (D.polish[b] != 0 ? 1 : 0) + 4 * (D.polish[b] == 2 ? 1 : 0));
+    if (REST && (D.lean & 2)) {
+      const bool mg = P.hessian != OH_HESSIAN_HYBRID || (!restart && D.stat[b] <= P.hyb_switch);
+      const unsigned long long m = __ballot(mg);
+      if (m && (int)(threadIdx.x & 63) == __ffsll((long long)m) - 1) atomicAdd(D.work + 6, (unsigned long long)__popcll(m));
+    }
   }
 }
 template <int N>
@@ -420,10 +459,10 @@
   hipLaunchKernelGGL(k_couple<N>, dim3(nbx8 * (P.T - P.t0)), dim3(256), 0, s, P, D, slot);
 }
 template <int N>
-static void launch_step_t(hipStream_t s, const FigParams& P, const FigBuffers& D, int slot) {
+static void launch_step_t(hipStream_t s, const FigParams& P, const FigBuffers& D, int slot, bool with_copy) {
   if (P.zc) {
     hipLaunchKernelGGL(k_step_zc<N>, dim3((D.B + 63) / 64), dim3(64), 0, s, P, D, slot);
-    if (P.hessian != OH_HESSIAN_GAUSS_NEWTON) hipLaunchKernelGGL(k_defer_copy<N>, dim3(512), dim3(256), 0, s, P, D, slot);
+    if (P.hessian != OH_HESSIAN_GAUSS_NEWTON && with_copy) hipLaunchKernelGGL(k_defer_copy<N>, dim3(512), dim3(256), 0, s, P, D, slot);
   } else hipLaunchKernelGGL(k_step<N>, dim3((D.B + 63) / 64), dim3(64), 0, s, P, D, slot);
 }
 template <int N>
@@ -504,8 +543,19 @@
 #undef C
   return true;
 }
-bool oh_launch_step(hipStream_t s, int n, const FigParams& P, const FigBuffers& D, int slot) {
-#define C(NN) launch_step_t<NN>(s, P, D, slot)
+bool oh_launch_step(hipStream_t s, int n, const FigParams& P, const FigBuffers& D, int slot, bool with_copy) {
+#define C(NN) launch_step_t<NN>(s, P, D, slot, with_copy)
+  OH_DISPATCH_N(n, C)
+#undef C
+  return true;
+}
+bool oh_launch_sweep_lists(hipStream_t s, int n, const FigParams& P, const FigBuffers& D, int slot, bool rescue, int count) {
+  const int nk = P.T - P.t0;
+  const long long thr = count < 0 ? 512LL * 256 : (long long)count * nk;
+  const long long nb = (thr + 255) / 256;
+  const int blocks = nb > 512 ? 512 : (nb < 1 ? 1 : (int)nb);
+  const int resc = rescue ? 1 : 0;
+#define C(NN) hipLaunchKernelGGL(k_sweep_lists<NN>, dim3(blocks), dim3(256), 0, s, P, D, slot, resc)
   OH_DISPATCH_N(n, C)
 #undef C
   return true;
diff --git a/optas_amd/csrc/oh_types.h b/optas_amd/csrc/oh_types.h
--- a/optas_amd/csrc/oh_types.h
+++ b/optas_amd/csrc/oh_types.h
@@ -109,4 +109,8 @@
   unsigned long long* work;
   int* n_defer;
   int* defer_list;
+  int lean;
+  int* oldidx;
+  int* rescue_list;
+  int* n_rescue;
 };
```

Result: faster. 3.194 million solves/s (median of 6 runs) (+1.2%).
